# HI-ComputerVision/uni-encoder-code

Hardware: AMD Instinct MI355X
Metric: img/s fwd+bwd Swin-L 1024x2048 bs=2 per GPU (higher is better)
Workload: dtype bf16; 1 GPU; BASELINE configs[2]: full OneFormer (Swin-L ws12 backbone + MSDeformAttn pixel decoder + 150-query masked-attention decoder), 1024x2048, fwd+bwd, synthetic loss; global_batch=2, parallelism=dp1, mode=eval() (train_mode reported separately with --full)

## Files before the change

### include/uenc.h

```cpp
#ifndef UENC_H
#define UENC_H
#include <stdint.h>

#ifdef __cplusplus
extern "C" {
#endif

#define UENC_F32 0
#define UENC_BF16 1

#ifndef UENC_STREAM_T
#define UENC_STREAM_T void*
#endif
typedef UENC_STREAM_T uenc_stream_t;

#define UENC_EPI_NONE 0
#define UENC_EPI_GELU 1
#define UENC_EPI_RELU 2
#define UENC_EPI_RESIDUAL 3
#define UENC_EPI_MUL_DGELU 4
#define UENC_EPI_MUL_DRELU 5

int uenc_version(void);
const char* uenc_arch(void);

int uenc_cast_f32_bf16(const float* src, void* dst, long n , uenc_stream_t stream);
int uenc_dropout_bf16(const void* in, void* out, long n, unsigned seed, float p, uenc_stream_t stream);
int uenc_cast_transpose_f32_bf16(const float* src , void* dst , int R, int C, uenc_stream_t stream);

int uenc_cast_multi(const void* table, int n, long total_tiles, uenc_stream_t stream);

int uenc_upsample_bilinear(const float* in, float* out, long NC, int Hi, int Wi, int Ho, int Wo, uenc_stream_t stream);

int uenc_attn_mask(const float* logits, uint8_t* mask, long rows, int Hi, int Wi, int Ho, int Wo, uenc_stream_t stream);

int uenc_add_cast_bf16(const float* a, const float* b, void* out, long n, long period, uenc_stream_t stream);
int uenc_msda_prep_fwd(const float* offaw, long ld, const float* ref, int ref_per_image, const int64_t* shapes, float* loc,
                       float* aw, long rows, int Lq, int M, int L, int P, uenc_stream_t stream);
int uenc_msda_prep_bwd(const float* dloc, const float* daw, const float* aw, const int64_t* shapes, void* doffaw, long ld,
                       long rows, int Lq, int M, int L, int P, uenc_stream_t stream);
int uenc_segment_colsum(const void* x16, long ld, int cols, const int64_t* seg_start, int nseg, long rows_per_image, int images,
                        float* out, uenc_stream_t stream);

long uenc_groupnorm_tokens_scratch_bytes(int B, int HW, int C, int G);
int uenc_groupnorm_tokens_fwd(const void* x, int x_dtype, const float* gamma, const float* beta, void* y, int y_dtype,
                              float* stats, void* scratch, const float* add_src, int Hs, int Ws, int H, int W, int B, int HW,
                              int C, int G, float eps, int relu, uenc_stream_t stream);
int uenc_groupnorm_tokens_bwd(const void* dy, int dy_dtype, const void* x, int x_dtype, const float* gamma, const float* beta,
                              const float* stats, void* dx, int dx_dtype, float* dgamma, float* dbeta, void* scratch, int B,
                              int HW, int C, int G, int relu, uenc_stream_t stream);
int uenc_upsample_bilinear_tokens_bwd(const void* dy, int dy_dtype, float* dsrc, int B, int H, int W, int Hs, int Ws, int C,
                                      uenc_stream_t stream);
int uenc_im2col3x3(const void* in, void* col, int B, int H, int W, int C, uenc_stream_t stream);
int uenc_col2im3x3(const void* dcol, void* dx, int B, int H, int W, int C, uenc_stream_t stream);
int uenc_im2col3x3_s2(const void* in, void* col, int B, int H, int W, int C, uenc_stream_t stream);
int uenc_col2im3x3_s2(const void* dcol, float* dx, int B, int H, int W, int C, uenc_stream_t stream);

int uenc_gemm_nt(const void* A, int a_dtype, long lda, const void* W, long ldw, void* C, int c_dtype, long ldc,
                 int M, int N, int K, const float* bias, int epilogue, const void* aux, long ldaux,
                 void* aux_out, long ldaux_out, float alpha, int splitk, int accumulate, uenc_stream_t stream);
#define UENC_NT_TILE_256X256 256
#define UENC_NT_TILE_256X192 192
#define UENC_NT_TILE_128X256 128
int uenc_gemm_nt_tile(const void* A, int a_dtype, long lda, const void* W, long ldw, void* C, int c_dtype, long ldc,
                      int M, int N, int K, const float* bias, int epilogue, const void* aux, long ldaux,
                      void* aux_out, long ldaux_out, float alpha, int splitk, int accumulate, int tile, uenc_stream_t stream);
int uenc_gemm_nt_scaled(const void* A, int a_dtype, long lda, const void* W, long ldw, void* C, int c_dtype, long ldc,
                        int M, int N, int K, const float* bias, int epilogue, const void* aux, long ldaux,
                        void* aux_out, long ldaux_out, float alpha, const float* sample_scale, int rows_per_sample, uenc_stream_t stream);
int uenc_gemm_nt_ln(const void* A, int a_dtype, long lda, const void* W, long ldw, void* C, long ldc, int M, int N, int K, const float* bias,
                    const void* residual, long ldres, const float* gamma, const float* beta, float eps, float* y32, void* y16, float* stats,
                    uenc_stream_t stream);
int uenc_gemm_nt_splits(int K, int splitk);
int uenc_gemm_nt_partials(const void* A, int a_dtype, long lda, const void* W, long ldw, float* P, long ldp, long part_stride,
                          int M, int N, int K, float alpha, int splitk, uenc_stream_t stream);

int uenc_gemm_nt_batched(const void* A, int a_dtype, long lda, long bsA, const void* W, long ldw, long bsW, void* C, int c_dtype,
                         long ldc, long bsC, int batch, int M, int N, int K, float alpha, int splitk, int accumulate, uenc_stream_t stream);

int uenc_gemm_tn(const void* dY, int dy_dtype, long ldy, const void* X, int x_dtype, long ldx, float* dW, long ldw,
                 float* db, int M, int N, int K, int splitm, uenc_stream_t stream);
int uenc_gemm_tn_tile(const void* dY, int dy_dtype, long ldy, const void* X, int x_dtype, long ldx, float* dW, long ldw,
                      float* db, int M, int N, int K, int splitm, int tile, uenc_stream_t stream);
int uenc_gemm_tn_scaled(const void* dY, int dy_dtype, long ldy, const void* X, int x_dtype, long ldx, float* dW, long ldw,
                        float* db, int M, int N, int K, int splitm, float alpha, uenc_stream_t stream);

int uenc_gemm_tn_grouped(const void* table, int n, int total_items, int tile, double flops, uenc_stream_t stream);
int uenc_gemm_tn_grouped_small(const void* table, int n, int total_items, double flops, uenc_stream_t stream);

int uenc_layernorm_fwd(const void* x, int x_dtype, const void* res, int res_dtype, float* h_out, const float* gamma,
                       const float* beta, void* y, int y_dtype, float* stats, long M, int C, float eps, void* y16,
                       uenc_stream_t stream);
int uenc_layernorm_bwd(const void* dy, int dy_dtype, const void* h, int h_dtype, const float* stats, const float* gamma,
                       const float* dres, void* dx, int dx_dtype, float* dgamma, float* dbeta, long M, int C, void* dx16,
                       float* part_ws, int defer_param_sums, uenc_stream_t stream);
int uenc_layernorm_bwd_blocks(long M, int C);
int uenc_ln_param_grouped(const void* table, int n, int total_groups, uenc_stream_t stream);
int uenc_patch_merge_ln_fwd(const float* x, const float* gamma, const float* beta, void* y, float* stats, int B, int H, int W,
                            int C, float eps, uenc_stream_t stream);
int uenc_patch_merge_ln_bwd(const void* dy, int dy_dtype, const float* x, const float* stats, const float* gamma, float* dx,
                            float* dgamma, float* dbeta, float* part_ws, int B, int H, int W, int C, int defer_param_sums,
                            uenc_stream_t stream);

int uenc_window_attn_np(int ws);
int uenc_relpos_expand(const float* table , float* bias_q ,
                       float* bias_k , int nH, int ws, uenc_stream_t stream);
int uenc_relpos_expand_grouped(const void* table, int n, int total_blocks, uenc_stream_t stream);
int uenc_window_attn_fwd(const void* qkv, const void* qkv_bias, const float* bias_q, void* out, float* lse, int B, int H, int W,
                         int C, int nH, int ws, int shift, float scale, uenc_stream_t stream);
long uenc_window_attn_bwd_ws_floats(int B, int H, int W, int nH, int ws);
int uenc_window_attn_bwd(const void* qkv, const void* qkv_bias, const float* bias_q, const float* bias_k,
                         const void* o_saved, const float* lse , const void* d_out, void* dqkv,
                         float* dS_ws, float* dtable, float* dbias_pad,
                         int B, int H, int W, int C, int nH, int ws, int shift, float scale, int defer_dtable, uenc_stream_t stream);
int uenc_window_attn_bwd_groups(int B, int H, int W, int nH, int ws);
int uenc_window_attn_dtable_grouped(const void* table, int n, int total_blocks, uenc_stream_t stream);

int uenc_msdeform_attn_fwd(const void* value, int v_dtype, const int64_t* shapes, const int64_t* level_start,
                           const float* loc, const float* attn, void* out, int out_dtype, int B, int S, int M, int D,
                           int L, int Lq, int P, uenc_stream_t stream);
int uenc_msdeform_attn_fwd_tiled(const void* value, int v_dtype, const int64_t* shapes, const int64_t* level_start,
                                 const float* loc, const float* attn, void* out, int out_dtype, int B, int S, int M, int D,
                                 int L, int Lq, int P, const int64_t* shapes_host, uenc_stream_t stream);
int uenc_msdeform_attn_bwd(const void* value, int v_dtype, const int64_t* shapes, const int64_t* level_start,
                           const float* loc, const float* attn, const void* grad_out, int go_dtype, float* grad_value,
                           float* grad_loc, float* grad_attn, int B, int S, int M, int D, int L, int Lq, int P,
                           const int64_t* shapes_host, void* workspace, long workspace_bytes, uenc_stream_t stream);
long uenc_msdeform_attn_bwd_workspace_bytes(const int64_t* shapes_host, int B, int M, int D, int L, int Lq, int P);
int uenc_msdeform_attn_fused_fwd(const void* value, int v_dtype, const int64_t* shapes, const int64_t* level_start, const float* offaw,
                                 long ld, const float* ref, int ref_per_image, void* out, int out_dtype, int B, int S, int M, int D,
                                 int L, int Lq, int P, uenc_stream_t stream);
int uenc_msdeform_attn_fused_fwd_tiled(const void* value, int v_dtype, const int64_t* shapes, const int64_t* level_start, const float* offaw,
                                       long ld, const float* ref, int ref_per_image, void* out, int out_dtype, int B, int S, int M, int D,
                                       int L, int Lq, int P, const int64_t* shapes_host, uenc_stream_t stream);
int uenc_msdeform_attn_fused_bwd(const void* value, int v_dtype, const int64_t* shapes, const int64_t* level_start, const float* offaw,
                                 long ld, const float* ref, int ref_per_image, const void* grad_out, int go_dtype, float* grad_value,
                                 void* doffaw, long ld_doffaw, int B, int S, int M, int D, int L, int Lq, int P, const int64_t* shapes_host,
                                 void* workspace, long workspace_bytes, uenc_stream_t stream);

long uenc_mha_fwd_workspace_floats(int B, int H, int Lq, int S);
int uenc_mha_fwd(const void* q, long q_bs, long q_rs, const void* k, long k_bs, long k_rs, const void* v, long v_bs,
                 long v_rs, const unsigned char* mask, long mask_rs, void* out, long o_bs, long o_rs, float* lse,
                 float* workspace, int B, int H, int Lq, int S, float scale, float dropout_p, unsigned seed, uenc_stream_t stream);
int uenc_mha_bwd(const void* q, long q_bs, long q_rs, const void* k, long k_bs, long k_rs, const void* v, long v_bs,
                 long v_rs, const unsigned char* mask, long mask_rs, const void* out, long o_bs, long o_rs,
                 const float* lse, const void* dout, long do_bs, long do_rs, float* dq, long dq_bs, long dq_rs, void* dk,
                 long dk_bs, long dk_rs, void* dv, long dv_bs, long dv_rs, int B, int H, int Lq, int S, float scale,
                 float dropout_p, unsigned seed, uenc_stream_t stream);

int uenc_na2d_fwd(const void* qkv, const float* rpb, void* out, float* lse, int B, int H, int W, int nH, int K, int dilation,
                  float scale, uenc_stream_t stream);
int uenc_na2d_bwd(const void* qkv, const float* rpb, const void* out, const void* dout, const float* lse, void* dqkv, float* drpb,
                  float* delta_ws, int B, int H, int W, int nH, int K, int dilation, float scale, uenc_stream_t stream);

int uenc_postproc_semantic(const float* mask_logits, const float* class_prob, float* sem, int Q, int C, int Cp, int hl, int wl,
                           int Hp, int Wp, int Ho, int Wo, uenc_stream_t stream);
int uenc_postproc_panoptic_stats(const float* mask_logits, const float* score, int* ids, int* counts, int Q, int hl, int wl, int Hp,
                                 int Wp, int Ho, int Wo, uenc_stream_t stream);
int uenc_postproc_panoptic_label(const float* mask_logits, const int* ids, const int* segid, int* seg, int Q, int hl, int wl, int Hp,
                                 int Wp, int Ho, int Wo, uenc_stream_t stream);

int uenc_gemm_nt_f32(const float* A, long lda, const float* W, long ldw, float* C, long ldc, int M, int N, int K, const float* bias,
                     int epilogue, const float* aux, long ldaux, float* aux_out, long ldaux_out, float alpha, int accumulate, uenc_stream_t stream);
int uenc_gemm_tn_f32(const float* dY, long ldy, const float* X, long ldx, float* dW, long ldw, float* db, int M, int N, int K, uenc_stream_t stream);
int uenc_window_attn_f32_fwd(const float* qkv, const float* qkv_bias, const float* table, float* out, int B, int H, int W, int C, int nH,
                             int ws, int shift, float scale, uenc_stream_t stream);
int uenc_window_attn_f32_bwd(const float* qkv, const float* qkv_bias, const float* table, const float* dout, float* dqkv, float* dtable,
                             float* dbias_pad, int B, int H, int W, int C, int nH, int ws, int shift, float scale, uenc_stream_t stream);
int uenc_mha_f32_fwd(const float* q, long qs0, long qs1, const float* k, long ks0, long ks1, const float* v, long vs0, long vs1,
                     const uint8_t* mask, long mask_row_stride, float* out, long os0, long os1, float* lse, int B, int nH, int Lq, int S,
                     float scale, float dropout_p, unsigned seed, uenc_stream_t stream);
int uenc_mha_f32_bwd(const float* q, long qs0, long qs1, const float* k, long ks0, long ks1, const float* v, long vs0, long vs1,
                     const uint8_t* mask, long mask_row_stride, const float* out, long os0, long os1, const float* lse, const float* dout,
                     long gos0, long gos1, float* dq, long dqs0, long dqs1, float* dk, long dks0, long dks1, float* dv, long dvs0, long dvs1,
                     float* delta, int B, int nH, int Lq, int S, float scale, float dropout_p, unsigned seed, uenc_stream_t stream);
int uenc_na2d_f32_fwd(const float* qkv, const float* rpb, float* out, float* lse, int B, int H, int W, int nH, int K, int dilation,
                      float scale, uenc_stream_t stream);
int uenc_na2d_f32_bwd(const float* qkv, const float* rpb, const float* out, const float* dout, const float* lse, float* dqkv, float* drpb,
                      int B, int H, int W, int nH, int K, int dilation, float scale, uenc_stream_t stream);

// ... 74 lines not shown
```

### uni-encoder-code_amd/csrc/gemm.hip

```cpp
#include "common.h"
#include "prof.h"

#define BM 128
#define BN 128
#define BK 64
#define GEMM_THREADS 256

enum { EPI_NONE = 0, EPI_GELU = 1, EPI_RELU = 2, EPI_RESIDUAL = 3, EPI_MUL_DGELU = 4, EPI_MUL_DRELU = 5 };

struct GemmNT {
    const void* A; int a_f32; long lda;
    const bf16* W; long ldw;
    void* C; long ldc;
    const float* bias;
    const void* aux; long ldaux;
    bf16* aux_out; long ldaux_out;
    int M, N, K;
    int tiles_m, tiles_n;
    int klen;
    int atomic;
    int persist;
    float alpha;
    const float* sample_scale; float inv_rows;
    long part_stride;
    int splits;
    long bsA, bsW, bsC;
    const float* ln_gamma; const float* ln_beta; float* ln_y32; bf16* ln_y16; float2* ln_stats; float ln_eps;
};

__device__ __forceinline__ float nt_alpha(const GemmNT& p, int m) {
    return p.sample_scale == nullptr ? p.alpha : p.alpha * p.sample_scale[(int)(((float)m + 0.5f) * p.inv_rows)];
}

__device__ __forceinline__ int lds_off(int row, int chunk) { return row * 128 + ((chunk ^ ((row >> 1) & 7)) << 4); }

template <bool F32>
__device__ __forceinline__ u32x4 load_row8(const void* base, long ld, int row, int nrows, int k, int kend, int K) {
    const bool ok = (row < nrows) && (k < kend);
    const int rc = min(row, nrows - 1), kc = min(k, K - 8);
    u32x4 v;
    if (F32) {
        const float* p = (const float*)base + (long)rc * ld + kc;
        const float4 a = *(const float4*)p, b = *(const float4*)(p + 4);
        const bf16x8 r = cvt8(a, b);
        v = *(const u32x4*)&r;
    } else {
        v = *(const u32x4*)((const bf16*)base + (long)rc * ld + kc);
    }
    const u32x4 z = {0u, 0u, 0u, 0u};
    return ok ? v : z;
}

template <int EPI, int OUT_F32>
__global__ __launch_bounds__(GEMM_THREADS) void gemm_nt_kernel(GemmNT p) {
    __shared__ __attribute__((aligned(16))) unsigned char smem[2 * (BM + BN) * BK * 2];
    if (blockIdx.z > 0) {
        p.A = (const char*)p.A + (long)blockIdx.z * p.bsA * (p.a_f32 ? 4 : 2);
        p.W += (long)blockIdx.z * p.bsW;
        p.C = (char*)p.C + (long)blockIdx.z * p.bsC * (OUT_F32 ? 4 : 2);
    }
    if (OUT_F32 && p.part_stride > 0) p.C = (float*)p.C + (long)blockIdx.y * p.part_stride;
    const int t = threadIdx.x, lane = t & 63, wave = t >> 6;
    const int wm = wave >> 1, wn = wave & 1;
    const int tile = xcd_remap(blockIdx.x, gridDim.x);
    const int mt = tile / p.tiles_n, nt = tile - mt * p.tiles_n;
    const int m0 = mt * BM, n0 = nt * BN;
    const int kbeg = blockIdx.y * p.klen;
    const int kend = min(p.K, kbeg + p.klen);
    const int nkt = (kend - kbeg + BK - 1) / BK;

    f32x4 acc[4][4];
#pragma unroll
    for (int i = 0; i < 4; ++i)
#pragma unroll
        for (int j = 0; j < 4; ++j) acc[i][j] = (f32x4){0.f, 0.f, 0.f, 0.f};

    const int srow = t >> 3, schunk = t & 7;
    u32x4 ra[4], rw[4];
    auto gload = [&](int kt) {
        const int k = kbeg + kt * BK + schunk * 8;
#pragma unroll
        for (int i = 0; i < 4; ++i) rw[i] = load_row8<false>(p.W, p.ldw, n0 + srow + 32 * i, p.N, k, kend, p.K);
        if (p.a_f32) {
#pragma unroll
            for (int i = 0; i < 4; ++i) ra[i] = load_row8<true>(p.A, p.lda, m0 + srow + 32 * i, p.M, k, kend, p.K);
        } else {
#pragma unroll
            for (int i = 0; i < 4; ++i) ra[i] = load_row8<false>(p.A, p.lda, m0 + srow + 32 * i, p.M, k, kend, p.K);
        }
    };
    auto lstore = [&](int buf) {
        unsigned char* As = smem + buf * ((BM + BN) * BK * 2);
        unsigned char* Ws = As + BM * BK * 2;
#pragma unroll
        for (int i = 0; i < 4; ++i) {
            *(u32x4*)(As + lds_off(srow + 32 * i, schunk)) = ra[i];
            *(u32x4*)(Ws + lds_off(srow + 32 * i, schunk)) = rw[i];
        }
    };

    gload(0);
    lstore(0);
    __syncthreads();
    const int fr = lane & 15, fg = lane >> 4;
    for (int kt = 0; kt < nkt; ++kt) {
        const int buf = kt & 1;
        if (kt + 1 < nkt) gload(kt + 1);
        const unsigned char* As = smem + buf * ((BM + BN) * BK * 2);
        const unsigned char* Ws = As + BM * BK * 2;
#pragma unroll
        for (int ks = 0; ks < 2; ++ks) {
            bf16x8 wf[4], xf[4];
#pragma unroll
            for (int i = 0; i < 4; ++i) wf[i] = *(const bf16x8*)(Ws + lds_off(wn * 64 + i * 16 + fr, ks * 4 + fg));
#pragma unroll
            for (int j = 0; j < 4; ++j) xf[j] = *(const bf16x8*)(As + lds_off(wm * 64 + j * 16 + fr, ks * 4 + fg));
#pragma unroll
            for (int i = 0; i < 4; ++i)
#pragma unroll
                for (int j = 0; j < 4; ++j) acc[i][j] = mfma16(wf[i], xf[j], acc[i][j]);
        }
        if (kt + 1 < nkt) lstore(buf ^ 1);
        __syncthreads();
    }

    const bool lead = (blockIdx.y == 0);
    if (p.atomic) {
#pragma unroll
        for (int j = 0; j < 4; ++j) {
            const int m = m0 + wm * 64 + j * 16 + fr;
            if (m >= p.M) continue;
#pragma unroll
            for (int i = 0; i < 4; ++i) {
                const int n = n0 + wn * 64 + i * 16 + 4 * fg;
                if (n >= p.N) continue;
                float* c = (float*)p.C + (long)m * p.ldc + n;
#pragma unroll
                for (int r = 0; r < 4; ++r) {
                    float v = acc[i][j][r];
                    if (p.bias != nullptr && lead) v += p.bias[n + r];
                    atomicAdd(c + r, v * p.alpha);
                }
            }
        }
        return;
    }
    float* T = (float*)smem;
    constexpr int LDT = 132;
    const int erow = t >> 4, ecol = (t & 15) * 8;
#pragma unroll
    for (int h = 0; h < 2; ++h) {
        __syncthreads();
        if (wm == h) {
#pragma unroll
            for (int j = 0; j < 4; ++j)
#pragma unroll
                for (int i = 0; i < 4; ++i) *(f32x4*)(T + (j * 16 + fr) * LDT + wn * 64 + i * 16 + 4 * fg) = acc[i][j];
        }
        __syncthreads();
        const int n = n0 + ecol;
        if (n >= p.N) continue;
        const bool full8 = (n + 8 <= p.N);
        float bv[8] = {0.f, 0.f, 0.f, 0.f, 0.f, 0.f, 0.f, 0.f};
        if (p.bias != nullptr) {
            const float4 b0 = *(const float4*)(p.bias + n);
            bv[0] = b0.x; bv[1] = b0.y; bv[2] = b0.z; bv[3] = b0.w;
// ... 42 lines not shown
                    v[r] = (EPI == EPI_MUL_DGELU) ? v[r] * dgelu_f((float)sv[r]) : (((float)sv[r] > 0.f) ? v[r] : 0.f);
            }
            if (OUT_F32) {
                float* c = (float*)p.C + (long)m * p.ldc + n;
                *(float4*)c = make_float4(v[0], v[1], v[2], v[3]);
                if (full8) *(float4*)(c + 4) = make_float4(v[4], v[5], v[6], v[7]);
            } else {
                bf16x8 o;
#pragma unroll
                for (int r = 0; r < 8; ++r) o[r] = (bf16)v[r];
                bf16* c = (bf16*)p.C + (long)m * p.ldc + n;
                if (full8) *(bf16x8*)c = o;
                else { bf16x4 q4; q4[0] = o[0]; q4[1] = o[1]; q4[2] = o[2]; q4[3] = o[3]; *(bf16x4*)c = q4; }
            }
        }
    }
}


template <int EPI, int OUT_F32>
__device__ __forceinline__ void epilogue8(const GemmNT& p, int m, int n, bool full8, float (&v)[8]) {
    if (EPI == EPI_GELU) {
        if (p.aux_out != nullptr) {
            bf16x8 pre;
#pragma unroll
            for (int r = 0; r < 8; ++r) pre[r] = (bf16)v[r];
            bf16* dst = p.aux_out + (long)m * p.ldaux_out + n;
            if (full8) *(bf16x8*)dst = pre;
            else { bf16x4 q4; q4[0] = pre[0]; q4[1] = pre[1]; q4[2] = pre[2]; q4[3] = pre[3]; *(bf16x4*)dst = q4; }
        }
#pragma unroll
        for (int r = 0; r < 8; ++r) v[r] = gelu_f(v[r]);
    } else if (EPI == EPI_RELU) {
#pragma unroll
        for (int r = 0; r < 8; ++r) v[r] = fmaxf(v[r], 0.f);
    } else if (EPI == EPI_RESIDUAL) {
        const float* rp = (const float*)p.aux + (long)m * p.ldaux + n;
        const float4 r0 = *(const float4*)rp;
        v[0] += r0.x; v[1] += r0.y; v[2] += r0.z; v[3] += r0.w;
        if (full8) { const float4 r1 = *(const float4*)(rp + 4); v[4] += r1.x; v[5] += r1.y; v[6] += r1.z; v[7] += r1.w; }
    } else if (EPI == EPI_MUL_DGELU || EPI == EPI_MUL_DRELU) {
        const bf16* ap = (const bf16*)p.aux + (long)m * p.ldaux + n;
        bf16x8 sv;
        if (full8) sv = *(const bf16x8*)ap;
        else {
            const bf16x4 q4 = *(const bf16x4*)ap;
#pragma unroll
            for (int r = 0; r < 4; ++r) { sv[r] = q4[r]; sv[4 + r] = (bf16)0.f; }
        }
#pragma unroll
        for (int r = 0; r < 8; ++r)
            v[r] = (EPI == EPI_MUL_DGELU) ? v[r] * dgelu_f((float)sv[r]) : (((float)sv[r] > 0.f) ? v[r] : 0.f);
    }
    if (OUT_F32) {
        float* c = (float*)p.C + (long)m * p.ldc + n;
        *(float4*)c = make_float4(v[0], v[1], v[2], v[3]);
        if (full8) *(float4*)(c + 4) = make_float4(v[4], v[5], v[6], v[7]);
    } else {
        bf16x8 o;
#pragma unroll
        for (int r = 0; r < 8; ++r) o[r] = (bf16)v[r];
        bf16* c = (bf16*)p.C + (long)m * p.ldc + n;
        if (full8) *(bf16x8*)c = o;
        else { bf16x4 q4; q4[0] = o[0]; q4[1] = o[1]; q4[2] = o[2]; q4[3] = o[3]; *(bf16x4*)c = q4; }
    }
}

template <int EPI, int OUT_F32, int A_F32>
__global__ __launch_bounds__(256) void gemm_nt_skinny_kernel(GemmNT p) {
    constexpr int LDP = 68;
    __shared__ __attribute__((aligned(16))) float part[4 * 64 * LDP];
    const int t = threadIdx.x, lane = t & 63, wave = t >> 6;
    const int fr = lane & 15, fg = lane >> 4;
    const int mt = blockIdx.x / p.tiles_n, nt = blockIdx.x - mt * p.tiles_n;
    const int m0 = mt * 64, n0 = nt * 64;
    const int per = (((p.K + 31) >> 5) + 3) >> 2;
    const int kb = wave * per * 32, ke = min(p.K, kb + per * 32);

    f32x4 acc[4][4];
#pragma unroll
    for (int i = 0; i < 4; ++i)
#pragma unroll
        for (int j = 0; j < 4; ++j) acc[i][j] = (f32x4){0.f, 0.f, 0.f, 0.f};
    long aoff[4], woff[4];
#pragma unroll
    for (int j = 0; j < 4; ++j) {
        aoff[j] = (long)min(m0 + j * 16 + fr, p.M - 1) * p.lda;
        woff[j] = (long)min(n0 + j * 16 + fr, p.N - 1) * p.ldw;
    }
    const u32x4 z = {0u, 0u, 0u, 0u};
    for (int k = kb; k < ke; k += 128) {
        u32x4 xa[4][4], wa[4][4];
#pragma unroll
        for (int s = 0; s < 4; ++s) {
            const int kk = k + s * 32 + 8 * fg;
            const bool ok = kk < ke;
            const int kc = min(kk, p.K - 8);
#pragma unroll
            for (int j = 0; j < 4; ++j) {
                if (A_F32) {
                    const float* ap = (const float*)p.A + aoff[j] + kc;
                    const float4 a0 = *(const float4*)ap, a1 = *(const float4*)(ap + 4);
                    const bf16x8 r = cvt8(a0, a1);
                    xa[s][j] = ok ? *(const u32x4*)&r : z;
                } else {
                    const u32x4 v = *(const u32x4*)((const bf16*)p.A + aoff[j] + kc);
                    xa[s][j] = ok ? v : z;
                }
                const u32x4 w = *(const u32x4*)(p.W + woff[j] + kc);
                wa[s][j] = ok ? w : z;
            }
        }
#pragma unroll
        for (int s = 0; s < 4; ++s)
#pragma unroll
            for (int i = 0; i < 4; ++i)
#pragma unroll
                for (int j = 0; j < 4; ++j)
                    acc[i][j] = mfma16(*(const bf16x8*)&wa[s][i], *(const bf16x8*)&xa[s][j], acc[i][j]);
    }
    float* mine = part + wave * 64 * LDP;
#pragma unroll
    for (int j = 0; j < 4; ++j)
#pragma unroll
        for (int i = 0; i < 4; ++i) *(f32x4*)(mine + (j * 16 + fr) * LDP + i * 16 + 4 * fg) = acc[i][j];
    __syncthreads();
    const int row = t >> 2, m = m0 + row;
    if (m >= p.M) return;
#pragma unroll
    for (int h = 0; h < 2; ++h) {
        const int c = (t & 3) * 16 + h * 8, n = n0 + c;
        if (n >= p.N) continue;
        const bool full8 = (n + 8 <= p.N);
        float v[8] = {0.f, 0.f, 0.f, 0.f, 0.f, 0.f, 0.f, 0.f};
#pragma unroll
        for (int w = 0; w < 4; ++w) {
            const f32x4 a0 = *(const f32x4*)(part + (w * 64 + row) * LDP + c), a1 = *(const f32x4*)(part + (w * 64 + row) * LDP + c + 4);
#pragma unroll
            for (int r = 0; r < 4; ++r) { v[r] += a0[r]; v[4 + r] += a1[r]; }
        }
        if (p.bias != nullptr) {
            const float4 b0 = *(const float4*)(p.bias + n);
            v[0] += b0.x; v[1] += b0.y; v[2] += b0.z; v[3] += b0.w;
            if (full8) { const float4 b1 = *(const float4*)(p.bias + n + 4); v[4] += b1.x; v[5] += b1.y; v[6] += b1.z; v[7] += b1.w; }
        }
#pragma unroll
        for (int r = 0; r < 8; ++r) v[r] *= nt_alpha(p, m);
        epilogue8<EPI, OUT_F32>(p, m, n, full8, v);
    }
}

#define BM2 256
#define BN2 256
#define T2 512

__device__ __forceinline__ void wait_vmcnt_upto8(int n) {
    if (n >= 8) __builtin_amdgcn_s_waitcnt(0x0f78);
    else if (n == 7) __builtin_amdgcn_s_waitcnt(0x0f77);
    else if (n == 6) __builtin_amdgcn_s_waitcnt(0x0f76);
    else if (n == 5) __builtin_amdgcn_s_waitcnt(0x0f75);
    else if (n == 4) __builtin_amdgcn_s_waitcnt(0x0f74);
    else if (n == 3) __builtin_amdgcn_s_waitcnt(0x0f73);
    else if (n == 2) __builtin_amdgcn_s_waitcnt(0x0f72);
    else if (n == 1) __builtin_amdgcn_s_waitcnt(0x0f71);
    else __builtin_amdgcn_s_waitcnt(0x0f70);
}

template <int EPI, int NI = 4>
__device__ __forceinline__ void nt_epilogue_direct(const GemmNT& p, f32x4 (&acc)[4][8], int mbase, int nbase, int fr, int fg, bool lead) {
    static_assert(NI == 4 || NI == 3, "column groups per wave");
    constexpr int NP = NI / 2;
    constexpr bool ODD = (NI & 1) != 0;
    const int mrow = mbase + fr, ncol = nbase + 4 * fg;
    const int nodd = ncol + (NI - 1) * 16;
    float bv4[4][4];
#pragma unroll
    for (int i = 0; i < NI; ++i) {
        const int n = ncol + i * 16;
        float4 b = make_float4(0.f, 0.f, 0.f, 0.f);
        if (p.bias != nullptr && n < p.N && lead) b = *(const float4*)(p.bias + n);
        bv4[i][0] = b.x; bv4[i][1] = b.y; bv4[i][2] = b.z; bv4[i][3] = b.w;
    }
    const int odd = fg & 1;
    const int n16[2] = {nbase + (0 + odd) * 16 + 4 * (fg - odd), nbase + (2 + odd) * 16 + 4 * (fg - odd)};
    constexpr bool AUX16 = (EPI == EPI_MUL_DGELU || EPI == EPI_MUL_DRELU);
// ... 571 lines not shown
        unsigned char* As = smem + buf * STAGE3 + wave * 1024;
        unsigned char* Ws = As + BM3 * BK3 * 2;
#pragma unroll
        for (int q = 0; q < 2; ++q) __builtin_amdgcn_global_load_lds(asrc[q] + (long)ks * BK3, (lds_void*)(As + q * 4096), 16, 0, 0);
#pragma unroll
        for (int q = 0; q < 4; ++q) __builtin_amdgcn_global_load_lds(wsrc[q] + (long)ks * BK3, (lds_void*)(Ws + q * 4096), 16, 0, 0);
    };
    issue(0, 0);
    if (nks > 1) issue(1, 1);
    const int aoff = lds_off32(fr, fg), boff = lds_off32(wn * 64 + fr, fg);
    int buf = 0;
    for (int s = 0; s < nks; ++s) {
        if (s + 1 < nks) __builtin_amdgcn_s_waitcnt(0x0f76);
        else __builtin_amdgcn_s_waitcnt(0x0f70);
        __builtin_amdgcn_sched_barrier(0);
        __builtin_amdgcn_s_barrier();
        __builtin_amdgcn_sched_barrier(0);
        if (s + 2 < nks) issue(s + 2, buf == 0 ? 2 : buf - 1);
        const unsigned char* As = smem + buf * STAGE3;
        const unsigned char* Ws = As + BM3 * BK3 * 2;
        bf16x8 wf[4], xf[8];
#pragma unroll
        for (int i = 0; i < 4; ++i) wf[i] = *(const bf16x8*)(Ws + i * 1024 + boff);
#pragma unroll
        for (int j = 0; j < 8; ++j) xf[j] = *(const bf16x8*)(As + j * 1024 + aoff);
        __builtin_amdgcn_sched_barrier(0);
#pragma unroll
        for (int i = 0; i < 4; ++i)
#pragma unroll
            for (int j = 0; j < 8; ++j) acc[i][j] = mfma16(wf[i], xf[j], acc[i][j]);
        buf = buf == 2 ? 0 : buf + 1;
    }
    if (!OUT_F32) {
        nt_epilogue_direct<EPI>(p, acc, m0, n0 + wn * 64, fr, fg, true);
        return;
    }
    __syncthreads();
    nt_epilogue_staged<EPI, OUT_F32, T3, 1, 4, LN>(p, acc, smem, m0, n0, 0, wn, t, fr, fg, true);
}

template <int EPI, int OUT_F32, bool LN = false>
static int launch_nt128(GemmNT& p, hipStream_t stream) {
    p.tiles_m = (p.M + BM3 - 1) / BM3; p.tiles_n = (p.N + BN3 - 1) / BN3;
    static bool attr_set = false;
    if (!attr_set) {
        hipError_t e = hipFuncSetAttribute((const void*)gemm_nt128_kernel<EPI, OUT_F32, LN>, hipFuncAttributeMaxDynamicSharedMemorySize, 3 * STAGE3);
        if (e != hipSuccess) return (int)e;
        attr_set = true;
    }
    p.persist = 0;
    hipLaunchKernelGGL((gemm_nt128_kernel<EPI, OUT_F32, LN>), dim3(p.tiles_m * p.tiles_n), dim3(T3), 3 * STAGE3, stream, p);
    return UENC_OK;
}

static int nt_cu_count() {
    static int ncu = 0;
    if (ncu == 0) {
        int dev = 0, v = 0;
        if (hipGetDevice(&dev) == hipSuccess && hipDeviceGetAttribute(&v, hipDeviceAttributeMultiprocessorCount, dev) == hipSuccess && v >= 8) ncu = v / 8 * 8;
        else ncu = 256;
    }
    return ncu;
}

template <int EPI, int OUT_F32, int BNT = BN2, bool LN = false>
static int launch_nt256(GemmNT& p, hipStream_t stream) {
    p.tiles_m = (p.M + BM2 - 1) / BM2; p.tiles_n = (p.N + BNT - 1) / BNT;
    static bool attr_set = false;
    if (!attr_set) {
        hipError_t e = hipFuncSetAttribute((const void*)gemm_nt256_kernel<EPI, OUT_F32, BNT, LN>, hipFuncAttributeMaxDynamicSharedMemorySize, 131072);
        if (e != hipSuccess) return (int)e;
        attr_set = true;
    }
    const int ncu = nt_cu_count();
    const int ntiles = p.tiles_m * p.tiles_n;
    p.persist = (p.splits == 1 && ntiles > ncu) ? 1 : 0;
    hipLaunchKernelGGL((gemm_nt256_kernel<EPI, OUT_F32, BNT, LN>), dim3(p.persist ? ncu : ntiles, p.splits), dim3(T2), 131072, stream, p);
    return UENC_OK;
}

template <int EPI, int OUT_F32>
static int launch_nt_tile128(GemmNT& p, int batch, hipStream_t stream) {
    p.tiles_m = (p.M + BM - 1) / BM; p.tiles_n = (p.N + BN - 1) / BN;
    hipLaunchKernelGGL((gemm_nt_kernel<EPI, OUT_F32>), dim3(p.tiles_m * p.tiles_n, p.splits, batch), dim3(GEMM_THREADS), 0, stream, p);
    return UENC_OK;
}

template <int EPI, int OUT_F32>
static int launch_nt_skinny(GemmNT& p, hipStream_t stream) {
    p.tiles_m = (p.M + 63) / 64; p.tiles_n = (p.N + 63) / 64;
    const dim3 grid(p.tiles_m * p.tiles_n), block(GEMM_THREADS);
    if (p.a_f32) hipLaunchKernelGGL((gemm_nt_skinny_kernel<EPI, OUT_F32, 1>), grid, block, 0, stream, p);
    else hipLaunchKernelGGL((gemm_nt_skinny_kernel<EPI, OUT_F32, 0>), grid, block, 0, stream, p);
    return UENC_OK;
}

static bool nt192_wins(int M, int N) {
    const long ncu = nt_cu_count(), tm = (M + BM2 - 1) / BM2;
    const long r256 = (tm * ((N + 255) / 256) + ncu - 1) / ncu, r192 = (tm * ((N + 191) / 192) + ncu - 1) / ncu;
    return r192 * 90 < r256 * 100;
}

static bool nt128_wins(int M, int N, int K, int c_dtype) {
    if (c_dtype == UENC_BF16 && M > 200000) return false;
    return N > 192 && N <= 288 && K <= 1024;
}

enum NtRoute { NT_REFUSED = -1, NT_TILE128, NT_SKINNY, NT_HALF, NT_256, NT_192 };

static NtRoute nt_route(int M, int N, int K, int batch, int a_dtype, long lda, int c_dtype, int epilogue, bool summed, int klen, int splitk,
                        bool ln, int tile) {
    const bool prefer_half = tile == 0 ? nt128_wins(M, N, K, c_dtype) : tile == UENC_NT_TILE_128X256;
    const bool dma = batch == 1 && a_dtype == UENC_BF16 && K >= 128 && lda % 8 == 0 && N >= 192 && N % 8 == 0;
    const bool k32 = (K % BK != 0) && (K % BK3 == 0) && !summed && prefer_half;
    const long tiles256 = (long)((M + 255) / 256) * ((N + 255) / 256);
    const bool big = dma && ((K % BK == 0) || k32) &&
                     (summed ? (epilogue == EPI_NONE && c_dtype == UENC_F32 && klen % BK == 0 && tiles256 >= 4 && tiles256 * splitk >= 64) : tiles256 >= 160);
    const long htiles = (long)((M + 127) / 128) * ((N + 255) / 256);
    const bool mid = !big && dma && (K % BK == 0) && !summed && htiles >= 96 &&
                     (c_dtype == UENC_F32 ? (epilogue == EPI_NONE || epilogue == EPI_RESIDUAL || epilogue == EPI_RELU) : true);
    if (tile != 0 && !big) return NT_REFUSED;
    if (ln && !(big || mid)) return NT_REFUSED;
    const long tiles128 = (long)((M + BM - 1) / BM) * ((N + BN - 1) / BN);
    if (!big && batch == 1 && !summed && tiles128 <= 32 && K >= 64) return NT_SKINNY;
    if (!(big || mid)) return NT_TILE128;
    if (mid || (!summed && (K % BK3 == 0) && prefer_half)) return NT_HALF;
    if (tile == UENC_NT_TILE_128X256) return NT_REFUSED;
    const bool narrow_ok = !summed && !(ln && N > 192);
    if (tile == UENC_NT_TILE_256X192 && !narrow_ok) return NT_REFUSED;
    return narrow_ok && (tile == 0 ? nt192_wins(M, N) : tile == UENC_NT_TILE_256X192) ? NT_192 : NT_256;
}

template <int EPI, int OUT_F32>
static int launch_nt(NtRoute route, GemmNT& p, int batch, hipStream_t stream) {
    switch (route) {
        case NT_HALF: return launch_nt128<EPI, OUT_F32>(p, stream);
        case NT_256: return launch_nt256<EPI, OUT_F32>(p, stream);
        case NT_192: return launch_nt256<EPI, OUT_F32, 192>(p, stream);
        default: break;
    }
    if constexpr (EPI != EPI_RESIDUAL || OUT_F32) {
        if (route == NT_SKINNY) return launch_nt_skinny<EPI, OUT_F32>(p, stream);
        if (route == NT_TILE128) return launch_nt_tile128<EPI, OUT_F32>(p, batch, stream);
    }
    return UENC_EINVAL;
}

struct NtLn { const float* gamma; const float* beta; float* y32; void* y16; float* stats; float eps; };

static int gemm_nt_impl(const void* A, int a_dtype, long lda, const void* W, long ldw, void* C, int c_dtype, long ldc,
                        int M, int N, int K, const float* bias, int epilogue, const void* aux, long ldaux,
                        void* aux_out, long ldaux_out, float alpha, int splitk, int accumulate, int batch, long bsA, long bsW,
                        long bsC, hipStream_t stream, long part_stride = 0, const float* sample_scale = nullptr, int rows_per_sample = 0,
                        const NtLn* ln = nullptr, int tile = 0) {
    UENC_CHECK_ARG(A && W && C && M > 0 && N > 0 && K > 0);
    UENC_CHECK_ARG(a_dtype == UENC_F32 || a_dtype == UENC_BF16);
    UENC_CHECK_ARG(c_dtype == UENC_F32 || c_dtype == UENC_BF16);
    UENC_CHECK_ARG(K % 8 == 0 && N % 4 == 0 && ldw % 8 == 0 && ldc % 4 == 0);
    UENC_CHECK_ARG(a_dtype == UENC_F32 ? (lda % 4 == 0) : (lda % 8 == 0));
    UENC_CHECK_ARG(((uintptr_t)A & 15) == 0 && ((uintptr_t)W & 15) == 0 && ((uintptr_t)C & 15) == 0);
    UENC_CHECK_ARG(epilogue >= EPI_NONE && epilogue <= EPI_MUL_DRELU);
    UENC_CHECK_ARG(tile == 0 || tile == UENC_NT_TILE_256X256 || tile == UENC_NT_TILE_256X192 || tile == UENC_NT_TILE_128X256);
    if (epilogue >= EPI_RESIDUAL) UENC_CHECK_ARG(aux != nullptr && ldaux % 4 == 0);
    if (splitk < 1) splitk = 1;
    if (splitk > 1 || accumulate) UENC_CHECK_ARG(c_dtype == UENC_F32 && epilogue == EPI_NONE);
    GemmNT p;
    p.A = A; p.a_f32 = (a_dtype == UENC_F32); p.lda = lda;
    p.W = (const bf16*)W; p.ldw = ldw;
    p.C = C; p.ldc = ldc; p.bias = bias; p.aux = aux; p.ldaux = ldaux;
    p.aux_out = (bf16*)aux_out; p.ldaux_out = ldaux_out;
    p.M = M; p.N = N; p.K = K;
    p.tiles_m = 0; p.tiles_n = 0; p.persist = 0;
    const int kt = (K + BK - 1) / BK;
    if (splitk > kt) splitk = kt;
    p.klen = ((kt + splitk - 1) / splitk) * BK;
    splitk = (K + p.klen - 1) / p.klen;
    p.atomic = (splitk > 1 || accumulate) ? 1 : 0;
    p.part_stride = 0; p.splits = splitk;
    const bool partials = part_stride > 0;
    if (partials) {
        UENC_CHECK_ARG(c_dtype == UENC_F32 && epilogue == EPI_NONE && !accumulate && bias == nullptr && batch == 1 && part_stride % 4 == 0);
        p.atomic = 0; p.part_stride = part_stride;
    }
    p.alpha = alpha;
    p.sample_scale = nullptr; p.inv_rows = 0.f;
    if (sample_scale != nullptr) {
        UENC_CHECK_ARG(rows_per_sample > 0 && !p.atomic && !partials && batch == 1 && M < (1 << 22));
        p.sample_scale = sample_scale; p.inv_rows = 1.0f / (float)rows_per_sample;
    }
    p.bsA = bsA; p.bsW = bsW; p.bsC = bsC;
    p.ln_gamma = nullptr; p.ln_beta = nullptr; p.ln_y32 = nullptr; p.ln_y16 = nullptr; p.ln_stats = nullptr; p.ln_eps = 0.f;

    const bool summed = p.atomic || partials;
    const NtRoute route = nt_route(M, N, K, batch, a_dtype, lda, c_dtype, epilogue, summed, p.klen, splitk, ln != nullptr, tile);
    if (route == NT_REFUSED) return UENC_EINVAL;
    const bool dma_kernel = route == NT_HALF || route == NT_256 || route == NT_192;
    if (c_dtype == UENC_F32) UENC_CHECK_ARG(epilogue == EPI_NONE || epilogue == EPI_RESIDUAL || epilogue == EPI_RELU);
    else UENC_CHECK_ARG(epilogue != EPI_RESIDUAL || dma_kernel);
    if (ln != nullptr) {
        UENC_CHECK_ARG(epilogue == EPI_RESIDUAL && c_dtype == UENC_F32 && !summed && N <= 256 && N % 8 == 0 && ldc == N &&
                       ln->gamma && ln->beta && (ln->y32 || ln->y16));
        UENC_CHECK_ARG((((uintptr_t)ln->gamma | (uintptr_t)ln->beta | (uintptr_t)ln->y32 | (uintptr_t)ln->y16) & 15) == 0 && ((uintptr_t)ln->stats & 7) == 0);
        p.ln_gamma = ln->gamma; p.ln_beta = ln->beta; p.ln_y32 = ln->y32; p.ln_y16 = (bf16*)ln->y16; p.ln_stats = (float2*)ln->stats; p.ln_eps = ln->eps;
    }

    const bool prof = uenc_prof_on();
    if (prof) {
        const double mn = (double)M * N;
        double bytes = (double)M * K * (a_dtype == UENC_F32 ? 4 : 2) + (double)N * K * 2 + mn * (c_dtype == UENC_F32 ? 4 : 2);
        if (epilogue == EPI_RESIDUAL) bytes += mn * 4;
        if (epilogue == EPI_MUL_DGELU || epilogue == EPI_MUL_DRELU) bytes += mn * 2;
        if (aux_out != nullptr) bytes += mn * 2;
        uenc_prof_begin(route == NT_HALF ? UENC_PROF_GEMM_NT128 : dma_kernel ? UENC_PROF_GEMM_NT256 : UENC_PROF_GEMM_NT, 2.0 * batch * M * (double)N * K, stream,
                        batch * bytes);
    }
    int rc = UENC_EINVAL;
    if (ln != nullptr) {
        rc = route == NT_HALF ? launch_nt128<EPI_RESIDUAL, 1, true>(p, stream)
                              : route == NT_192 ? launch_nt256<EPI_RESIDUAL, 1, 192, true>(p, stream) : launch_nt256<EPI_RESIDUAL, 1, BN2, true>(p, stream);
    } else {
        switch (epilogue * 2 + (c_dtype == UENC_F32 ? 1 : 0)) {
#define NT_CASE(E, F) case (E) * 2 + (F): rc = launch_nt<E, F>(route, p, batch, stream); break
            NT_CASE(EPI_NONE, 1); NT_CASE(EPI_RESIDUAL, 1); NT_CASE(EPI_RELU, 1);
            NT_CASE(EPI_NONE, 0); NT_CASE(EPI_GELU, 0); NT_CASE(EPI_RELU, 0); NT_CASE(EPI_MUL_DGELU, 0); NT_CASE(EPI_MUL_DRELU, 0);
            NT_CASE(EPI_RESIDUAL, 0);
#undef NT_CASE
            default: break;
        }
    }
    if (prof) uenc_prof_end(stream);
    if (rc != UENC_OK) return rc;
    UENC_LAUNCH_RET();
}

extern "C" int uenc_gemm_nt(const void* A, int a_dtype, long lda, const void* W, long ldw, void* C, int c_dtype, long ldc,
                            int M, int N, int K, const float* bias, int epilogue, const void* aux, long ldaux,
                            void* aux_out, long ldaux_out, float alpha, int splitk, int accumulate, hipStream_t stream) {
    return gemm_nt_impl(A, a_dtype, lda, W, ldw, C, c_dtype, ldc, M, N, K, bias, epilogue, aux, ldaux, aux_out, ldaux_out, alpha, splitk,
                        accumulate, 1, 0, 0, 0, stream);
}

extern "C" int uenc_gemm_nt_tile(const void* A, int a_dtype, long lda, const void* W, long ldw, void* C, int c_dtype, long ldc,
                                 int M, int N, int K, const float* bias, int epilogue, const void* aux, long ldaux,
                                 void* aux_out, long ldaux_out, float alpha, int splitk, int accumulate, int tile, hipStream_t stream) {
    return gemm_nt_impl(A, a_dtype, lda, W, ldw, C, c_dtype, ldc, M, N, K, bias, epilogue, aux, ldaux, aux_out, ldaux_out, alpha, splitk,
                        accumulate, 1, 0, 0, 0, stream, 0, nullptr, 0, nullptr, tile);
}

extern "C" int uenc_gemm_nt_scaled(const void* A, int a_dtype, long lda, const void* W, long ldw, void* C, int c_dtype, long ldc,
                                   int M, int N, int K, const float* bias, int epilogue, const void* aux, long ldaux,
                                   void* aux_out, long ldaux_out, float alpha, const float* sample_scale, int rows_per_sample,
                                   hipStream_t stream) {
    UENC_CHECK_ARG(sample_scale != nullptr && rows_per_sample > 0);
    return gemm_nt_impl(A, a_dtype, lda, W, ldw, C, c_dtype, ldc, M, N, K, bias, epilogue, aux, ldaux, aux_out, ldaux_out, alpha, 1,
                        0, 1, 0, 0, 0, stream, 0, sample_scale, rows_per_sample);
}

extern "C" int uenc_gemm_nt_ln(const void* A, int a_dtype, long lda, const void* W, long ldw, void* C, long ldc, int M, int N, int K, const float* bias,
                               const void* residual, long ldres, const float* gamma, const float* beta, float eps, float* y32, void* y16, float* stats,
                               hipStream_t stream) {
    UENC_CHECK_ARG(residual != nullptr);
    NtLn ln = {gamma, beta, y32, y16, stats, eps};
    return gemm_nt_impl(A, a_dtype, lda, W, ldw, C, UENC_F32, ldc, M, N, K, bias, EPI_RESIDUAL, residual, ldres, nullptr, 0, 1.0f, 1, 0, 1, 0, 0, 0, stream, 0,
                        nullptr, 0, &ln);
}

extern "C" int uenc_gemm_nt_splits(int K, int splitk) {
    const int kt = (K + BK - 1) / BK;
    if (splitk < 1) splitk = 1;
    if (splitk > kt) splitk = kt;
    const int klen = (kt + splitk - 1) / splitk;
    return (kt + klen - 1) / klen;
}

extern "C" int uenc_gemm_nt_partials(const void* A, int a_dtype, long lda, const void* W, long ldw, float* P, long ldp, long part_stride,
                                     int M, int N, int K, float alpha, int splitk, hipStream_t stream) {
    UENC_CHECK_ARG(splitk >= 1 && uenc_gemm_nt_splits(K, splitk) == splitk && part_stride >= (long)(M - 1) * ldp + N);
    return gemm_nt_impl(A, a_dtype, lda, W, ldw, P, UENC_F32, ldp, M, N, K, nullptr, EPI_NONE, nullptr, 0, nullptr, 0, alpha, splitk, 0, 1, 0, 0,
                        0, stream, part_stride);
}

extern "C" int uenc_gemm_nt_batched(const void* A, int a_dtype, long lda, long bsA, const void* W, long ldw, long bsW, void* C, int c_dtype,
                                    long ldc, long bsC, int batch, int M, int N, int K, float alpha, int splitk, int accumulate,
                                    hipStream_t stream) {
    UENC_CHECK_ARG(batch >= 1 && batch <= 65535);
    UENC_CHECK_ARG((bsA * (a_dtype == UENC_F32 ? 4 : 2)) % 16 == 0 && (bsW * 2) % 16 == 0 && (bsC * (c_dtype == UENC_F32 ? 4 : 2)) % 16 == 0);
    return gemm_nt_impl(A, a_dtype, lda, W, ldw, C, c_dtype, ldc, M, N, K, nullptr, EPI_NONE, nullptr, 0, nullptr, 0, alpha, splitk, accumulate,
                        batch, bsA, bsW, bsC, stream);
}

struct GemmTN {
    const void* dY; int dy_f32; long ldy;
    const void* X; int x_f32; long ldx;
    float* dW; long ldw;
    float* db;
    int M, N, K;
    int tiles_n, tiles_k;
    int mlen;
    int store;
    float alpha;
};

__device__ __forceinline__ void transpose8x8(const u32x4 (&in)[8], u32x4 (&out)[8]) {
#pragma unroll
    for (int c = 0; c < 8; ++c) {
#pragma unroll
        for (int w = 0; w < 4; ++w) {
            const unsigned lo = in[2 * w][c >> 1], hi = in[2 * w + 1][c >> 1];
            out[c][w] = __builtin_amdgcn_perm(hi, lo, (c & 1) ? 0x07060302u : 0x05040100u);
        }
    }
}

__device__ __forceinline__ void tn_small_body(const GemmTN& p, int tile, int msplit) {
    __shared__ __attribute__((aligned(16))) unsigned char smem[2 * (BM + BN) * BK * 2];
    const int t = threadIdx.x, lane = t & 63, wave = t >> 6;
    const int wk = wave >> 1, wn = wave & 1;
    const int ntile = tile / p.tiles_k, ktile = tile - ntile * p.tiles_k;
    const int n0 = ntile * BN, k0 = ktile * BM;
    const int mbeg = msplit * p.mlen;
    const int mend = min(p.M, mbeg + p.mlen);
    const int nit = (mend - mbeg + BK - 1) / BK;
// ... 424 lines not shown
```

### uni-encoder-code_amd/csrc/layernorm.hip

```cpp
#include "common.h"
#include <stdlib.h>

struct LnFwd {
    const void* x; int x_f32;
    const void* res; int res_f32;
    float* h_out;
    const float* gamma; const float* beta;
    void* y; int y_f32;
    bf16* y16;
    float2* stats;
    long M; int C; float eps;
    int mgH, mgW, mgC;
};

struct PatchGather {
    long base; bool ok[4];
    __device__ __forceinline__ PatchGather(long row, int H, int W, int C) {
        const int W2 = (W + 1) >> 1, H2 = (H + 1) >> 1;
        const int j = (int)(row % W2);
        const long r2 = row / W2;
        const int i = (int)(r2 % H2);
        const long b = r2 / H2;
        base = ((b * H + 2 * i) * W + 2 * j) * C;
        const bool y1 = 2 * i + 1 < H, x1 = 2 * j + 1 < W;
// ... 270 lines not shown
}

extern "C" int uenc_layernorm_bwd_blocks(long M, int C) {
    if (M <= 0 || C <= 0) return 0;
    bool stored = false;
    const long b = ln_bwd_blocks(M, C, true, &stored);
    return stored ? (int)b : 0;
}

static int ln_bwd_launch(LnBwd& p, float* part_ws, int defer, hipStream_t stream) {
    const long M = p.M; const int C = p.C;
    float* dgamma = p.dgamma; float* dbeta = p.dbeta;
    bool stored = false;
    const long blocks = ln_bwd_blocks(M, C, part_ws != nullptr && dgamma != nullptr, &stored);
    p.part = stored ? part_ws : nullptr;
    const int nv = (C + 255) / 256;
    const size_t shm = (size_t)(C > 2048 ? 1 : 4) * 2 * C * sizeof(float);
    dim3 grid((unsigned)blocks), block(256);
    if (nv <= 1) LN_LAUNCH(bwd, 1, grid, block, shm, stream, p);
    else if (nv <= 2) LN_LAUNCH(bwd, 2, grid, block, shm, stream, p);
    else if (nv <= 4) LN_LAUNCH(bwd, 4, grid, block, shm, stream, p);
    else if (nv <= 8) LN_LAUNCH(bwd, 8, grid, block, shm, stream, p);
    else if (nv <= 16) LN_LAUNCH(bwd, 16, grid, block, shm, stream, p);
    else LN_LAUNCH(bwd, 24, grid, block, shm, stream, p);
    if (p.part != nullptr && !defer)
        hipLaunchKernelGGL(ln_bwd_param_kernel, dim3((2 * C + 63) / 64, 16), dim3(256), 0, stream, (const float*)p.part, (int)blocks, C, dgamma, dbeta);
    UENC_LAUNCH_RET();
}

struct LnParamDesc { const float* part; float* dgamma; float* dbeta; int nblk, C, group_begin, pad; };
__global__ __launch_bounds__(256) void ln_param_grouped_kernel(const LnParamDesc* __restrict__ table, int n) {
    __shared__ float red[4][64];
    int lo = 0, hi = n - 1;
    const int grp = blockIdx.x;
    while (lo < hi) {
        const int mid = (lo + hi + 1) >> 1;
        if (table[mid].group_begin <= grp) lo = mid; else hi = mid - 1;
    }
    const LnParamDesc d = table[lo];
    const int C = d.C, nblk = d.nblk;
    const int col = (grp - d.group_begin) * 64 + (threadIdx.x & 63), r = threadIdx.x >> 6;
    const int per = (nblk + gridDim.y - 1) / gridDim.y, b0 = blockIdx.y * per, b1 = min(nblk, b0 + per);
    float acc = 0.f;
    if (col < 2 * C)
        for (int b = b0 + r; b < b1; b += 4) acc += d.part[(long)b * 2 * C + col];
    red[r][threadIdx.x & 63] = acc;
    __syncthreads();
    if (r == 0 && col < 2 * C) {
        const float v = red[0][threadIdx.x] + red[1][threadIdx.x] + red[2][threadIdx.x] + red[3][threadIdx.x];
        atomicAdd(col < C ? d.dgamma + col : d.dbeta + (col - C), v);
    }
}

extern "C" int uenc_ln_param_grouped(const void* table, int n, int total_groups, hipStream_t stream) {
    UENC_CHECK_ARG(table && n > 0 && total_groups > 0 && ((uintptr_t)table & 7) == 0);
    static_assert(sizeof(LnParamDesc) == 40, "descriptor layout is part of the ABI");
    hipLaunchKernelGGL(ln_param_grouped_kernel, dim3((unsigned)total_groups, 16), dim3(256), 0, stream, (const LnParamDesc*)table, n);
    UENC_LAUNCH_RET();
}


extern "C" int uenc_patch_merge_ln_fwd(const float* x, const float* gamma, const float* beta, void* y, float* stats, int B, int H, int W,
                                       int C, float eps, hipStream_t stream) {
    UENC_CHECK_ARG(x && gamma && beta && y && stats && B > 0 && H > 0 && W > 0 && C > 0 && C % 4 == 0 && 4 * C <= 6144);
    UENC_CHECK_ARG((((uintptr_t)x | (uintptr_t)y) & 15) == 0);
    LnFwd p;
    p.x = x; p.x_f32 = 1; p.res = nullptr; p.res_f32 = 0; p.h_out = nullptr; p.gamma = gamma; p.beta = beta; p.y = y; p.y_f32 = 0;
    p.y16 = nullptr; p.stats = (float2*)stats; p.M = (long)B * ((H + 1) / 2) * ((W + 1) / 2); p.C = 4 * C; p.eps = eps;
    p.mgH = H; p.mgW = W; p.mgC = C;
    return ln_fwd_launch(p, stream);
}

extern "C" int uenc_patch_merge_ln_bwd(const void* dy, int dy_dtype, const float* x, const float* stats, const float* gamma, float* dx,
                                       float* dgamma, float* dbeta, float* part_ws, int B, int H, int W, int C, int defer_param_sums,
                                       hipStream_t stream) {
    UENC_CHECK_ARG(dy && x && stats && gamma && dx && B > 0 && H > 0 && W > 0 && C > 0 && C % 4 == 0 && 4 * C <= 6144);
    UENC_CHECK_ARG((dgamma == nullptr) == (dbeta == nullptr));
    LnBwd p;
    p.dy = dy; p.dy_f32 = (dy_dtype == UENC_F32); p.h = x; p.h_f32 = 1; p.stats = (const float2*)stats; p.gamma = gamma; p.dres = nullptr;
    p.dx = dx; p.dx_f32 = 1; p.dx16 = nullptr; p.dgamma = dgamma; p.dbeta = dbeta;
    p.M = (long)B * ((H + 1) / 2) * ((W + 1) / 2); p.C = 4 * C; p.mgH = H; p.mgW = W; p.mgC = C;
    return ln_bwd_launch(p, part_ws, defer_param_sums, stream);
}
```

### uni-encoder-code_amd/uenc/attention.py

```python
from typing import Optional

import torch

from . import kernels as K
from .capi import check, lib, stream_ptr


def _strided(t: torch.Tensor) -> torch.Tensor:
    if t.dtype != K.adt():
        t = t.to(K.adt())
    if t.stride(2) != 1 or t.stride(1) % 8 or t.stride(0) % 8 or t.data_ptr() % 16:
        t = t.contiguous()
    return t


def _mask_bytes(mask: Optional[torch.Tensor]):
    if mask is None:
        return None, 0
    m = mask.to(torch.uint8) if mask.dtype != torch.bool else mask.view(torch.uint8)
    S = m.shape[-1]
    if S % 4 or not m.is_contiguous():
        Sp = -(-S // 4) * 4
        m = torch.nn.functional.pad(m, (0, Sp - S)).contiguous()
    return m, m.shape[-1]


class MHACoreFn(torch.autograd.Function):
    @staticmethod
    def forward(ctx, q, k, v, nheads, mask, dropout_p=0.0, seed=0):
        q, k, v = _strided(q), _strided(k), _strided(v)
        B, Lq, E = q.shape
        S = k.shape[1]
        assert E == nheads * 32, "the HIP attention kernels are built for head_dim 32"
        scale = 32 ** -0.5
        m8, mrs = _mask_bytes(mask)
        lse = torch.empty((B, nheads, Lq), dtype=torch.float32, device=q.device)
        if K.EXACT:
            if isinstance(seed, K.SeedSlot):
                raise RuntimeError("device-side dropout seeds (ops.device_rng) are not available in the fp32 exact mode")
            out = torch.empty((B, Lq, E), dtype=torch.float32, device=q.device)
            check(lib.uenc_mha_f32_fwd(q.data_ptr(), q.stride(0), q.stride(1), k.data_ptr(), k.stride(0), k.stride(1),
                                       v.data_ptr(), v.stride(0), v.stride(1), m8.data_ptr() if m8 is not None else 0, mrs,
                                       out.data_ptr(), out.stride(0), out.stride(1), lse.data_ptr(), B, nheads, Lq, S, scale, float(dropout_p), int(seed),
                                       stream_ptr()), "mha_f32_fwd")
            ctx.save_for_backward(q, k, v, out, lse, m8 if m8 is not None else torch.empty(0, device=q.device))
            ctx.meta = (nheads, S, scale, mrs, m8 is not None, float(dropout_p), int(seed))
            return out
        out = torch.empty((B, Lq, E), dtype=torch.bfloat16, device=q.device)
        nws = lib.uenc_mha_fwd_workspace_floats(B, nheads, Lq, S)
        ws = torch.empty((nws,), dtype=torch.float32, device=q.device) if nws else None
        args = (q.data_ptr(), q.stride(0), q.stride(1), k.data_ptr(), k.stride(0), k.stride(1),
                v.data_ptr(), v.stride(0), v.stride(1), m8.data_ptr() if m8 is not None else 0, mrs,
                out.data_ptr(), out.stride(0), out.stride(1), lse.data_ptr(),
                ws.data_ptr() if ws is not None else 0, B, nheads, Lq, S, scale, float(dropout_p))
        if isinstance(seed, K.SeedSlot):
            check(lib.uenc_mha_fwd_sp(*args, seed.seeds.data_ptr(), seed.slot, stream_ptr()), "mha_fwd_sp")
        else:
            check(lib.uenc_mha_fwd(*args, int(seed), stream_ptr()), "mha_fwd")
        ctx.save_for_backward(q, k, v, out, lse, m8 if m8 is not None else torch.empty(0, device=q.device))
        ctx.meta = (nheads, S, scale, mrs, m8 is not None, float(dropout_p), seed if isinstance(seed, K.SeedSlot) else int(seed))
        return out

    @staticmethod
    def backward(ctx, dout):
        q, k, v, out, lse, m8 = ctx.saved_tensors
        nheads, S, scale, mrs, has_mask, dropout_p, seed = ctx.meta
        B, Lq, E = q.shape
        dout = _strided(dout)
        if K.EXACT:
            dq = torch.empty((B, Lq, E), dtype=torch.float32, device=q.device)
            dk = torch.zeros((B, S, E), dtype=torch.float32, device=q.device)
            dv = torch.zeros((B, S, E), dtype=torch.float32, device=q.device)
            delta = torch.empty((B, nheads, Lq), dtype=torch.float32, device=q.device)
            check(lib.uenc_mha_f32_bwd(q.data_ptr(), q.stride(0), q.stride(1), k.data_ptr(), k.stride(0), k.stride(1),
                                       v.data_ptr(), v.stride(0), v.stride(1), m8.data_ptr() if has_mask else 0, mrs,
                                       out.data_ptr(), out.stride(0), out.stride(1), lse.data_ptr(),
                                       dout.data_ptr(), dout.stride(0), dout.stride(1),
                                       dq.data_ptr(), dq.stride(0), dq.stride(1), dk.data_ptr(), dk.stride(0), dk.stride(1),
                                       dv.data_ptr(), dv.stride(0), dv.stride(1), delta.data_ptr(), B, nheads, Lq, S, scale, dropout_p, seed,
                                       stream_ptr()), "mha_f32_bwd")
            return dq, dk, dv, None, None, None, None
        dq = torch.zeros((B, Lq, E), dtype=torch.float32, device=q.device)
        dk = torch.empty((B, S, E), dtype=torch.bfloat16, device=q.device)
        dv = torch.empty((B, S, E), dtype=torch.bfloat16, device=q.device)
        args = (q.data_ptr(), q.stride(0), q.stride(1), k.data_ptr(), k.stride(0), k.stride(1),
                v.data_ptr(), v.stride(0), v.stride(1), m8.data_ptr() if has_mask else 0, mrs,
                out.data_ptr(), out.stride(0), out.stride(1), lse.data_ptr(),
                dout.data_ptr(), dout.stride(0), dout.stride(1),
                dq.data_ptr(), dq.stride(0), dq.stride(1), dk.data_ptr(), dk.stride(0), dk.stride(1),
                dv.data_ptr(), dv.stride(0), dv.stride(1), B, nheads, Lq, S, scale, dropout_p)
        if isinstance(seed, K.SeedSlot):
            seed.check()
            check(lib.uenc_mha_bwd_sp(*args, seed.seeds.data_ptr(), seed.slot, stream_ptr()), "mha_bwd_sp")
        else:
            check(lib.uenc_mha_bwd(*args, seed, stream_ptr()), "mha_bwd")
        return dq.to(torch.bfloat16), dk, dv, None, None, None, None


def mha(q, k, v, nheads: int, mask: Optional[torch.Tensor] = None, dropout_p: float = 0.0, seed: int = 0):
    if not q.is_cuda:
        raise RuntimeError("uenc attention runs on the GPU only")
    return MHACoreFn.apply(q, k, v, nheads, mask, dropout_p, seed)


def keep_mask_reference(B: int, nheads: int, Lq: int, S: int, dropout_p: float, seed: int) -> torch.Tensor:
    idx = torch.arange(B * nheads * Lq * S, dtype=torch.int64)
    M = 0xFFFFFFFF
    x = (((idx & M) ^ (((idx >> 32) * 0x9E3779B9) & M)) + seed) & M
    x = x ^ (x >> 16); x = (x * 0x7feb352d) & M
    x = x ^ (x >> 15); x = (x * 0x846ca68b) & M
    x = x ^ (x >> 16)
    thresh = 0 if dropout_p <= 0 else int(float(torch.tensor(dropout_p, dtype=torch.float32)) * 4294967296.0)
    return (x >= thresh).view(B, nheads, Lq, S)
```

### uni-encoder-code_amd/uenc/capi.py

```python
import ctypes
import os

import torch

_HERE = os.path.dirname(os.path.abspath(__file__))
LIB_PATH = os.path.join(_HERE, "libuenc_hip.so")

F32, BF16 = 0, 1
EPI_NONE, EPI_GELU, EPI_RELU, EPI_RESIDUAL, EPI_MUL_DGELU, EPI_MUL_DRELU = range(6)

c_p, c_i, c_l, c_f, c_u, c_d = ctypes.c_void_p, ctypes.c_int, ctypes.c_long, ctypes.c_float, ctypes.c_uint, ctypes.c_double

_SIGNATURES = {
    "uenc_version": [],
    "uenc_prof_enable": [c_i],
    "uenc_prof_collect": [c_i, c_p, c_p, c_p],
    "uenc_prof_collect_bytes": [c_i, c_p],
    "uenc_prof_next_bytes": [ctypes.c_double],
    "uenc_cast_f32_bf16": [c_p, c_p, c_l, c_p],
    "uenc_cast_transpose_f32_bf16": [c_p, c_p, c_i, c_i, c_p],
    "uenc_cast_multi": [c_p, c_i, c_l, c_p],
    "uenc_upsample_bilinear": [c_p, c_p, c_l, c_i, c_i, c_i, c_i, c_p],
    "uenc_attn_mask": [c_p, c_p, c_l, c_i, c_i, c_i, c_i, c_p],
    "uenc_gemm_nt": [c_p, c_i, c_l, c_p, c_l, c_p, c_i, c_l, c_i, c_i, c_i, c_p, c_i, c_p, c_l, c_p, c_l, c_f, c_i, c_i, c_p],
    "uenc_gemm_nt_tile": [c_p, c_i, c_l, c_p, c_l, c_p, c_i, c_l, c_i, c_i, c_i, c_p, c_i, c_p, c_l, c_p, c_l, c_f, c_i, c_i, c_i, c_p],
    "uenc_gemm_nt_scaled": [c_p, c_i, c_l, c_p, c_l, c_p, c_i, c_l, c_i, c_i, c_i, c_p, c_i, c_p, c_l, c_p, c_l, c_f, c_p, c_i, c_p],
    "uenc_gemm_nt_ln": [c_p, c_i, c_l, c_p, c_l, c_p, c_l, c_i, c_i, c_i, c_p, c_p, c_l, c_p, c_p, c_f, c_p, c_p, c_p, c_p],
    "uenc_groupnorm_tokens_scratch_bytes": [c_i, c_i, c_i, c_i],
    "uenc_groupnorm_tokens_fwd": [c_p, c_i, c_p, c_p, c_p, c_i, c_p, c_p, c_p, c_i, c_i, c_i, c_i, c_i, c_i, c_i, c_i, c_f, c_i, c_p],
    "uenc_groupnorm_tokens_bwd": [c_p, c_i, c_p, c_i, c_p, c_p, c_p, c_p, c_i, c_p, c_p, c_p, c_i, c_i, c_i, c_i, c_i, c_p],
    "uenc_upsample_bilinear_tokens_bwd": [c_p, c_i, c_p, c_i, c_i, c_i, c_i, c_i, c_i, c_p],
    "uenc_im2col3x3": [c_p, c_p, c_i, c_i, c_i, c_i, c_p],
    "uenc_col2im3x3": [c_p, c_p, c_i, c_i, c_i, c_i, c_p],
    "uenc_add_cast_bf16": [c_p, c_p, c_p, c_l, c_l, c_p],
    "uenc_msda_prep_fwd": [c_p, c_l, c_p, c_i, c_p, c_p, c_p, c_l, c_i, c_i, c_i, c_i, c_p],
    "uenc_msda_prep_bwd": [c_p, c_p, c_p, c_p, c_p, c_l, c_l, c_i, c_i, c_i, c_i, c_p],
    "uenc_segment_colsum": [c_p, c_l, c_i, c_p, c_i, c_l, c_i, c_p, c_p],
    "uenc_dropout_bf16": [c_p, c_p, c_l, c_u, c_f, c_p],
    "uenc_gemm_nt_splits": [c_i, c_i],
    "uenc_gemm_nt_partials": [c_p, c_i, c_l, c_p, c_l, c_p, c_l, c_l, c_i, c_i, c_i, c_f, c_i, c_p],
    "uenc_gemm_nt_batched": [c_p, c_i, c_l, c_l, c_p, c_l, c_l, c_p, c_i, c_l, c_l, c_i, c_i, c_i, c_i, c_f, c_i, c_i, c_p],
    "uenc_gemm_tn": [c_p, c_i, c_l, c_p, c_i, c_l, c_p, c_l, c_p, c_i, c_i, c_i, c_i, c_p],
    "uenc_gemm_tn_tile": [c_p, c_i, c_l, c_p, c_i, c_l, c_p, c_l, c_p, c_i, c_i, c_i, c_i, c_i, c_p],
    "uenc_gemm_tn_scaled": [c_p, c_i, c_l, c_p, c_i, c_l, c_p, c_l, c_p, c_i, c_i, c_i, c_i, c_f, c_p],
    "uenc_gemm_tn_grouped": [c_p, c_i, c_i, c_i, ctypes.c_double, c_p],
    "uenc_gemm_tn_grouped_small": [c_p, c_i, c_i, ctypes.c_double, c_p],
    "uenc_layernorm_fwd": [c_p, c_i, c_p, c_i, c_p, c_p, c_p, c_p, c_i, c_p, c_l, c_i, c_f, c_p, c_p],
    "uenc_layernorm_bwd": [c_p, c_i, c_p, c_i, c_p, c_p, c_p, c_p, c_i, c_p, c_p, c_l, c_i, c_p, c_p, c_i, c_p],
    "uenc_layernorm_bwd_blocks": [c_l, c_i],
    "uenc_ln_param_grouped": [c_p, c_i, c_i, c_p],
    "uenc_window_attn_bwd_groups": [c_i, c_i, c_i, c_i, c_i],
    "uenc_window_attn_dtable_grouped": [c_p, c_i, c_i, c_p],
    "uenc_msdeform_attn_fwd": [c_p, c_i, c_p, c_p, c_p, c_p, c_p, c_i, c_i, c_i, c_i, c_i, c_i, c_i, c_i, c_p],
    "uenc_msdeform_attn_fwd_tiled": [c_p, c_i, c_p, c_p, c_p, c_p, c_p, c_i, c_i, c_i, c_i, c_i, c_i, c_i, c_i, c_p, c_p],
    "uenc_msdeform_attn_bwd": [c_p, c_i, c_p, c_p, c_p, c_p, c_p, c_i, c_p, c_p, c_p, c_i, c_i, c_i, c_i, c_i, c_i, c_i, c_p, c_p, c_l, c_p],
    "uenc_msdeform_attn_bwd_workspace_bytes": [c_p, c_i, c_i, c_i, c_i, c_i, c_i],
    "uenc_msdeform_attn_fused_fwd": [c_p, c_i, c_p, c_p, c_p, c_l, c_p, c_i, c_p, c_i, c_i, c_i, c_i, c_i, c_i, c_i, c_i, c_p],
    "uenc_msdeform_attn_fused_fwd_tiled": [c_p, c_i, c_p, c_p, c_p, c_l, c_p, c_i, c_p, c_i, c_i, c_i, c_i, c_i, c_i, c_i, c_i, c_p, c_p],
    "uenc_msdeform_attn_fused_bwd": [c_p, c_i, c_p, c_p, c_p, c_l, c_p, c_i, c_p, c_i, c_p, c_p, c_l, c_i, c_i, c_i, c_i, c_i, c_i, c_i, c_p, c_p, c_l, c_p],
    "uenc_mha_fwd_workspace_floats": [c_i, c_i, c_i, c_i],
    "uenc_mha_fwd": [c_p, c_l, c_l, c_p, c_l, c_l, c_p, c_l, c_l, c_p, c_l, c_p, c_l, c_l, c_p, c_p, c_i, c_i, c_i, c_i, c_f, c_f, c_u, c_p],
    "uenc_mha_bwd": [c_p, c_l, c_l, c_p, c_l, c_l, c_p, c_l, c_l, c_p, c_l, c_p, c_l, c_l, c_p, c_p, c_l, c_l, c_p, c_l, c_l,
                     c_p, c_l, c_l, c_p, c_l, c_l, c_i, c_i, c_i, c_i, c_f, c_f, c_u, c_p],
    "uenc_window_attn_np": [c_i],
    "uenc_relpos_expand": [c_p, c_p, c_p, c_i, c_i, c_p],
    "uenc_relpos_expand_grouped": [c_p, c_i, c_i, c_p],
    "uenc_window_attn_fwd": [c_p, c_p, c_p, c_p, c_p, c_i, c_i, c_i, c_i, c_i, c_i, c_i, c_f, c_p],
    "uenc_postproc_semantic": [c_p, c_p, c_p, c_i, c_i, c_i, c_i, c_i, c_i, c_i, c_i, c_i, c_p],
    "uenc_postproc_panoptic_stats": [c_p, c_p, c_p, c_p, c_i, c_i, c_i, c_i, c_i, c_i, c_i, c_p],
    "uenc_postproc_panoptic_label": [c_p, c_p, c_p, c_p, c_i, c_i, c_i, c_i, c_i, c_i, c_i, c_p],
    "uenc_patch_merge_ln_fwd": [c_p, c_p, c_p, c_p, c_p, c_i, c_i, c_i, c_i, c_f, c_p],
    "uenc_patch_merge_ln_bwd": [c_p, c_i, c_p, c_p, c_p, c_p, c_p, c_p, c_p, c_i, c_i, c_i, c_i, c_i, c_p],
    "uenc_im2col3x3_s2": [c_p, c_p, c_i, c_i, c_i, c_i, c_p],
    "uenc_col2im3x3_s2": [c_p, c_p, c_i, c_i, c_i, c_i, c_p],
    "uenc_na2d_fwd": [c_p, c_p, c_p, c_p, c_i, c_i, c_i, c_i, c_i, c_i, c_f, c_p],
    "uenc_na2d_bwd": [c_p, c_p, c_p, c_p, c_p, c_p, c_p, c_p, c_i, c_i, c_i, c_i, c_i, c_i, c_f, c_p],
    "uenc_window_attn_bwd_ws_floats": [c_i, c_i, c_i, c_i, c_i],
    "uenc_step_rng_advance": [c_p, c_p, c_i, c_i, c_p, c_i, c_p, c_i, c_p],
    "uenc_dropout_sp": [c_p, c_p, c_l, c_i, c_p, c_i, c_f, c_p],
    "uenc_upload": [c_p, c_p, c_l, c_p],
    "uenc_prof_active": [],
    "uenc_scale_rows_bf16": [c_p, c_l, c_p, c_l, c_l, c_i, c_p, c_l, c_p],
    "uenc_mha_fwd_sp": [c_p, c_l, c_l, c_p, c_l, c_l, c_p, c_l, c_l, c_p, c_l, c_p, c_l, c_l, c_p, c_p, c_i, c_i, c_i, c_i, c_f, c_f, c_p, c_i, c_p],
    "uenc_mha_bwd_sp": [c_p, c_l, c_l, c_p, c_l, c_l, c_p, c_l, c_l, c_p, c_l, c_p, c_l, c_l, c_p, c_p, c_l, c_l, c_p, c_l, c_l,
                        c_p, c_l, c_l, c_p, c_l, c_l, c_i, c_i, c_i, c_i, c_f, c_f, c_p, c_i, c_p],
    "uenc_gemm_nt_f32": [c_p, c_l, c_p, c_l, c_p, c_l, c_i, c_i, c_i, c_p, c_i, c_p, c_l, c_p, c_l, c_f, c_i, c_p],
    "uenc_gemm_tn_f32": [c_p, c_l, c_p, c_l, c_p, c_l, c_p, c_i, c_i, c_i, c_p],
    "uenc_window_attn_f32_fwd": [c_p, c_p, c_p, c_p, c_i, c_i, c_i, c_i, c_i, c_i, c_i, c_f, c_p],
    "uenc_window_attn_f32_bwd": [c_p, c_p, c_p, c_p, c_p, c_p, c_p, c_i, c_i, c_i, c_i, c_i, c_i, c_i, c_f, c_p],
    "uenc_mha_f32_fwd": [c_p, c_l, c_l, c_p, c_l, c_l, c_p, c_l, c_l, c_p, c_l, c_p, c_l, c_l, c_p, c_i, c_i, c_i, c_i, c_f, c_f, c_u, c_p],
    "uenc_mha_f32_bwd": [c_p, c_l, c_l, c_p, c_l, c_l, c_p, c_l, c_l, c_p, c_l, c_p, c_l, c_l, c_p, c_p, c_l, c_l, c_p, c_l, c_l,
                         c_p, c_l, c_l, c_p, c_l, c_l, c_p, c_i, c_i, c_i, c_i, c_f, c_f, c_u, c_p],
    "uenc_na2d_f32_fwd": [c_p, c_p, c_p, c_p, c_i, c_i, c_i, c_i, c_i, c_i, c_f, c_p],
    "uenc_na2d_f32_bwd": [c_p, c_p, c_p, c_p, c_p, c_p, c_p, c_i, c_i, c_i, c_i, c_i, c_i, c_f, c_p],
    "uenc_window_attn_bwd": [c_p, c_p, c_p, c_p, c_p, c_p, c_p, c_p, c_p, c_p, c_p, c_i, c_i, c_i, c_i, c_i, c_i, c_i, c_f, c_i, c_p],
    "uenc_optim_advance": [c_p, c_d, c_d, c_p],
    "uenc_optim_grad_sqnorm": [c_p, c_i, c_l, c_p, c_i, c_p, c_f, c_p],
    "uenc_optim_adamw_step": [c_p, c_i, c_l, c_p, c_i, c_p, c_d, c_d, c_d, c_p],
    "uenc_match_cost_workspace_floats": [c_i, c_i, c_i, c_i],
    "uenc_match_cost": [c_p, c_i, c_i, c_i, c_i, c_i, c_i, c_i, c_i, c_i, c_f, c_f, c_f, c_f, c_p, c_l, c_p, c_p],
    "uenc_lsap_solve": [c_p, c_i, c_i, c_p],
    "uenc_view_synth_workspace_floats": [c_i, c_i, c_i, c_i, c_i],
    "uenc_view_synth_fwd": [c_p, c_i, c_i, c_i, c_i, c_i, c_i, c_p],
    "uenc_view_synth_bwd": [c_p, c_i, c_i, c_i, c_i, c_i, c_i, c_p, c_l, c_p],
    "uenc_photo_loss_workspace_floats": [c_i, c_i, c_i, c_i],
    "uenc_photo_loss_fwd": [c_p, c_p, c_p, c_p, c_i, c_i, c_i, c_i, c_i, c_i, c_p, c_l, c_p, c_p, c_p],
    "uenc_photo_loss_bwd": [c_p, c_p, c_p, c_p, c_i, c_i, c_i, c_i, c_i, c_i, c_p, c_p],
    "uenc_dwconv7_ln_fwd": [c_p, c_p, c_p, c_p, c_p, c_p, c_p, c_i, c_p, c_i, c_i, c_i, c_i, c_f, c_p],
    "uenc_dwconv7_ln_bwd_data": [c_p, c_i, c_p, c_p, c_p, c_p, c_p, c_p, c_p, c_p, c_p, c_p, c_i, c_i, c_i, c_i, c_i, c_p],
    "uenc_dwconv7_bwd_weight_workspace_bytes": [c_i, c_i, c_i, c_i],
    "uenc_dwconv7_bwd_weight": [c_p, c_p, c_p, c_p, c_p, c_l, c_i, c_i, c_i, c_i, c_p],
    "uenc_layer_scale_grads": [c_p, c_p, c_p, c_p, c_p, c_p, c_p, c_p, c_i, c_i, c_p],
    "uenc_stem7x7_s2_patches": [c_p, c_p, c_i, c_i, c_i, c_i, c_p],
    "uenc_maxpool3x3_s2_fwd": [c_p, c_p, c_p, c_i, c_i, c_i, c_i, c_i, c_p],
    "uenc_maxpool3x3_s2_bwd": [c_p, c_p, c_p, c_i, c_i, c_i, c_i, c_i, c_p],
    "uenc_bn_workspace_floats": [c_l, c_i],
    "uenc_bn_stats": [c_p, c_i, c_l, c_i, c_p, c_p, c_p, c_p, c_p, c_f, c_p, c_l, c_p],
    "uenc_bn_act_fwd": [c_p, c_i, c_p, c_p, c_p, c_p, c_p, c_i, c_p, c_i, c_l, c_i, c_f, c_i, c_p],
    "uenc_bn_act_bwd_reduce": [c_p, c_i, c_p, c_i, c_p, c_i, c_p, c_p, c_l, c_i, c_f, c_i, c_p, c_p, c_p, c_p, c_l, c_p],
    "uenc_bn_act_bwd_apply": [c_p, c_i, c_p, c_i, c_p, c_i, c_p, c_p, c_p, c_p, c_p, c_i, c_p, c_i, c_l, c_i, c_f, c_i, c_i, c_p],
}


class UencError(RuntimeError):
    pass


def _load():
    if not os.path.exists(LIB_PATH):
        raise ImportError(
            f"{LIB_PATH} is missing: build it with `python -c 'import __graft_entry__ as g; g.build()'` "
            "(or `make -C uni-encoder-code_amd/csrc`). The HIP library is mandatory; there is no fallback path.")
# ... 49 lines not shown
```

### uni-encoder-code_amd/uenc/kernels.py

```python
import ctypes
import os
from typing import Optional

import torch

from . import capi
from .capi import BF16, F32, check, dt, lib, ptr, stream_ptr

EPI_NONE, EPI_GELU, EPI_RELU, EPI_RESIDUAL, EPI_MUL_DGELU, EPI_MUL_DRELU = (
    capi.EPI_NONE, capi.EPI_GELU, capi.EPI_RELU, capi.EPI_RESIDUAL, capi.EPI_MUL_DGELU, capi.EPI_MUL_DRELU)
NT_TILE_256X256, NT_TILE_256X192, NT_TILE_128X256 = 256, 192, 128


EXACT = os.environ.get("UENC_EXACT", "0") == "1"


def adt():
    return torch.float32 if EXACT else torch.bfloat16


def _odt(dtype):
    return torch.float32 if (EXACT and dtype == torch.bfloat16) else dtype


# ... 117 lines not shown
    x = _mix32_np(key, np.uint64(1 << 41) | idx).reshape(nb, n_samples)
    dp = (np.float32(1.0) - kp).astype(np.float32)
    thresh = np.array([0 if d <= 0 else (0xFFFFFFFF if d >= 1 else int(float(d) * 4294967296.0)) for d in dp], dtype=np.uint64)
    keep = (kp[:, None] > 0) & (x >= thresh[:, None])
    inv = (np.float32(1.0) / np.where(kp > 0, kp, np.float32(1.0))).astype(np.float32)
    scales = np.where(keep, inv[:, None], np.float32(0.0)).astype(np.float32)
    return scales, seeds


def cast_bf16(src: torch.Tensor, out: Optional[torch.Tensor] = None) -> torch.Tensor:
    assert src.dtype == torch.float32 and src.is_contiguous() and src.is_cuda
    if EXACT:
        return src if out is None else out.copy_(src)
    if out is None:
        out = torch.empty(src.shape, dtype=torch.bfloat16, device=src.device)
    n = src.numel()
    if n % 8 == 0 and src.data_ptr() % 16 == 0:
        check(lib.uenc_cast_f32_bf16(src.data_ptr(), out.data_ptr(), n, stream_ptr()), "cast_f32_bf16")
    else:
        check(lib.uenc_cast_transpose_f32_bf16(src.data_ptr(), out.data_ptr(), 1, n, stream_ptr()), "cast_f32_bf16")
    return out


def cast_transpose_bf16(src: torch.Tensor, out: Optional[torch.Tensor] = None) -> torch.Tensor:
    assert src.dtype == torch.float32 and src.dim() == 2 and src.is_contiguous() and src.is_cuda
    R, C = src.shape
    if EXACT:
        return src.t().contiguous() if out is None else out.copy_(src.t())
    if out is None:
        out = torch.empty((C, R), dtype=torch.bfloat16, device=src.device)
    assert out.dtype == torch.bfloat16 and tuple(out.shape) == (C, R) and out.is_contiguous()
    check(lib.uenc_cast_transpose_f32_bf16(src.data_ptr(), out.data_ptr(), R, C, stream_ptr()), "cast_transpose")
    return out


def gemm_nt(a: torch.Tensor, w: torch.Tensor, *, bias: Optional[torch.Tensor] = None, epilogue: int = EPI_NONE,
            aux: Optional[torch.Tensor] = None, aux_out: Optional[torch.Tensor] = None,
            out: Optional[torch.Tensor] = None, out_dtype=torch.bfloat16, alpha: float = 1.0,
            splitk: int = 1, accumulate: bool = False, sample_scale: Optional[torch.Tensor] = None, rows_per_sample: int = 0,
            tile: int = 0) -> torch.Tensor:
    _mat(a, "a"); _mat(w, "w")
    M, K = a.shape
    N, K2 = w.shape
    if EXACT:
        if sample_scale is not None:
            raise capi.UencError("gemm_nt: the fp32 verification kernels take no per-sample scale")
        return _gemm_nt_exact(a, w, bias, epilogue, aux, aux_out, out, alpha, accumulate)
    if K != K2 or w.dtype != torch.bfloat16:
        raise capi.UencError(f"gemm_nt: a {tuple(a.shape)} vs w {tuple(w.shape)} / {w.dtype}")
    if out is None:
        out = torch.empty((M, N), dtype=out_dtype, device=a.device)
        if splitk > 1 or accumulate:
            out.zero_()
    _mat(out, "out")
    assert out.shape == (M, N)
    if bias is not None:
        assert bias.dtype == torch.float32 and bias.numel() == N and bias.is_contiguous()
    if aux is not None:
        _mat(aux, "aux"); assert aux.shape == (M, N)
        assert aux.dtype == (torch.float32 if epilogue == EPI_RESIDUAL else torch.bfloat16)
    if aux_out is not None:
        _mat(aux_out, "aux_out"); assert aux_out.shape == (M, N) and aux_out.dtype == torch.bfloat16
    if sample_scale is not None:
        assert sample_scale.dtype == torch.float32 and sample_scale.is_cuda and sample_scale.is_contiguous()
        assert rows_per_sample > 0 and sample_scale.numel() * rows_per_sample >= M and splitk == 1 and not accumulate and tile == 0
        check(lib.uenc_gemm_nt_scaled(a.data_ptr(), dt(a), a.stride(0), w.data_ptr(), w.stride(0), out.data_ptr(), dt(out),
                                      out.stride(0), M, N, K, ptr(bias), epilogue, ptr(aux), aux.stride(0) if aux is not None else 0,
                                      ptr(aux_out), aux_out.stride(0) if aux_out is not None else 0, float(alpha), sample_scale.data_ptr(),
                                      int(rows_per_sample), stream_ptr()), "gemm_nt_scaled")
        return out
    if tile != 0:
        check(lib.uenc_gemm_nt_tile(a.data_ptr(), dt(a), a.stride(0), w.data_ptr(), w.stride(0), out.data_ptr(), dt(out),
                                    out.stride(0), M, N, K, ptr(bias), epilogue, ptr(aux), aux.stride(0) if aux is not None else 0,
                                    ptr(aux_out), aux_out.stride(0) if aux_out is not None else 0, float(alpha), int(splitk),
                                    int(accumulate), int(tile), stream_ptr()), "gemm_nt_tile")
        return out
    check(lib.uenc_gemm_nt(a.data_ptr(), dt(a), a.stride(0), w.data_ptr(), w.stride(0), out.data_ptr(), dt(out),
                           out.stride(0), M, N, K, ptr(bias), epilogue, ptr(aux), aux.stride(0) if aux is not None else 0,
                           ptr(aux_out), aux_out.stride(0) if aux_out is not None else 0, float(alpha), int(splitk),
                           int(accumulate), stream_ptr()), "gemm_nt")
    return out


def _gemm_nt_exact(a, w, bias, epilogue, aux, aux_out, out, alpha, accumulate) -> torch.Tensor:
    M, K = a.shape
    N, K2 = w.shape
    f32 = torch.float32
    if K != K2 or a.dtype != f32 or w.dtype != f32:
        raise capi.UencError(f"gemm_nt (exact): a {tuple(a.shape)} {a.dtype} vs w {tuple(w.shape)} {w.dtype}")
    if out is None:
        out = torch.zeros((M, N), dtype=f32, device=a.device) if accumulate else torch.empty((M, N), dtype=f32, device=a.device)
    _mat(out, "out")
    assert out.shape == (M, N) and out.dtype == f32
    for t, name in ((aux, "aux"), (aux_out, "aux_out")):
        if t is not None:
            _mat(t, name); assert t.shape == (M, N) and t.dtype == f32
    if bias is not None:
        assert bias.dtype == f32 and bias.numel() == N and bias.is_contiguous()
    check(lib.uenc_gemm_nt_f32(a.data_ptr(), a.stride(0), w.data_ptr(), w.stride(0), out.data_ptr(), out.stride(0), M, N, K, ptr(bias),
                               epilogue, ptr(aux), aux.stride(0) if aux is not None else 0, ptr(aux_out),
                               aux_out.stride(0) if aux_out is not None else 0, float(alpha), int(accumulate), stream_ptr()), "gemm_nt_f32")
    return out


def gemm_nt_splitk(a: torch.Tensor, w: torch.Tensor, splitk: int, *, alpha: float = 1.0) -> torch.Tensor:
    _mat(a, "a"); _mat(w, "w")
    M, K = a.shape
    N, K2 = w.shape
    if EXACT:
        return _gemm_nt_exact(a, w, None, EPI_NONE, None, None, None, alpha, False)
    if K != K2 or w.dtype != torch.bfloat16:
        raise capi.UencError(f"gemm_nt_splitk: a {tuple(a.shape)} vs w {tuple(w.shape)} / {w.dtype}")
    s = lib.uenc_gemm_nt_splits(K, int(splitk))
    part = torch.empty((s, M, N), dtype=torch.float32, device=a.device)
    check(lib.uenc_gemm_nt_partials(a.data_ptr(), dt(a), a.stride(0), w.data_ptr(), w.stride(0), part.data_ptr(), N, M * N, M, N, K,
                                    float(alpha), s, stream_ptr()), "gemm_nt_partials")
    return part[0] if s == 1 else part.sum(0)


def gemm_nt_batched(a: torch.Tensor, w: torch.Tensor, out: torch.Tensor, *, alpha: float = 1.0, splitk: int = 1, accumulate: bool = False):
    B, M, K = a.shape
    _, N, _ = w.shape
    if EXACT:
        for b in range(B):
            _gemm_nt_exact(a[b], w[b], None, EPI_NONE, None, None, out[b], alpha, accumulate or splitk > 1)
        return out
    assert a.is_cuda and w.dtype == torch.bfloat16 and w.shape == (B, N, K) and out.shape == (B, M, N)
    assert a.stride(2) == 1 and w.stride(2) == 1 and out.stride(2) == 1
    check(lib.uenc_gemm_nt_batched(a.data_ptr(), dt(a), a.stride(1), a.stride(0), w.data_ptr(), w.stride(1), w.stride(0), out.data_ptr(), dt(out),
                                   out.stride(1), out.stride(0), B, M, N, K, float(alpha), int(splitk), int(accumulate), stream_ptr()),
          "gemm_nt_batched")
    return out


def gemm_tn(dy: torch.Tensor, x: torch.Tensor, dw: torch.Tensor, db: Optional[torch.Tensor] = None, splitm: int = 0, alpha: float = 1.0,
            tile: int = 0):
    _mat(dy, "dy"); _mat(x, "x"); _mat(dw, "dw")
    M, N = dy.shape
    M2, K = x.shape
    if M != M2 or dw.dtype != torch.float32 or dw.shape != (N, K):
        raise capi.UencError(f"gemm_tn: dy {tuple(dy.shape)} x {tuple(x.shape)} dw {tuple(dw.shape)}")
    if db is not None:
        assert db.dtype == torch.float32 and db.numel() == N and db.is_contiguous()
    if EXACT:
        assert dy.dtype == torch.float32 and x.dtype == torch.float32 and alpha == 1.0
        check(lib.uenc_gemm_tn_f32(dy.data_ptr(), dy.stride(0), x.data_ptr(), x.stride(0), dw.data_ptr(), dw.stride(0), ptr(db), M, N, K,
                                   stream_ptr()), "gemm_tn_f32")
        return
    if alpha != 1.0:
        assert tile == 0
        check(lib.uenc_gemm_tn_scaled(dy.data_ptr(), dt(dy), dy.stride(0), x.data_ptr(), dt(x), x.stride(0), dw.data_ptr(), dw.stride(0),
                                      ptr(db), M, N, K, int(splitm), float(alpha), stream_ptr()), "gemm_tn_scaled")
        return
    if tile != 0:
        check(lib.uenc_gemm_tn_tile(dy.data_ptr(), dt(dy), dy.stride(0), x.data_ptr(), dt(x), x.stride(0), dw.data_ptr(), dw.stride(0),
                                    ptr(db), M, N, K, int(splitm), int(tile), stream_ptr()), "gemm_tn_tile")
        return
    check(lib.uenc_gemm_tn(dy.data_ptr(), dt(dy), dy.stride(0), x.data_ptr(), dt(x), x.stride(0), dw.data_ptr(), dw.stride(0),
                           ptr(db), M, N, K, int(splitm), stream_ptr()), "gemm_tn")


def gemm_nt_ln(a: torch.Tensor, w: torch.Tensor, bias: Optional[torch.Tensor], residual: torch.Tensor, gamma: torch.Tensor, beta: torch.Tensor,
               eps: float = 1e-5, want_y32: bool = True, want_y16: bool = True):
    M, Kd = a.shape
    N = w.shape[0]
    if (EXACT or a.dtype != torch.bfloat16 or N > 256 or N % 8 or Kd % 64 or os.environ.get("UENC_GEMM_LN", "1") == "0"
            or not (a.stride(1) == 1 and w.stride(1) == 1 and residual.is_contiguous() and residual.dtype == torch.float32)):
        return None
    h = torch.empty((M, N), dtype=torch.float32, device=a.device)
    y32 = torch.empty((M, N), dtype=torch.float32, device=a.device) if want_y32 else None
    y16 = torch.empty((M, N), dtype=torch.bfloat16, device=a.device) if want_y16 else None
    stats = torch.empty((M, 2), dtype=torch.float32, device=a.device)
    rc = lib.uenc_gemm_nt_ln(a.data_ptr(), dt(a), a.stride(0), w.data_ptr(), w.stride(0), h.data_ptr(), N, M, N, Kd, ptr(bias), residual.data_ptr(), N,
                             gamma.data_ptr(), beta.data_ptr(), float(eps), ptr(y32), ptr(y16), stats.data_ptr(), stream_ptr())
    if rc == -1:
        return None
    check(rc, "gemm_nt_ln")
    return h, y32, y16, stats


def layernorm_fwd(x: torch.Tensor, gamma: torch.Tensor, beta: torch.Tensor, *, res: Optional[torch.Tensor] = None,
                  out_dtype=torch.bfloat16, want_h: bool = False, want_stats: bool = True, eps: float = 1e-5,
                  twin: Optional[list] = None):
    C = x.shape[-1]
    assert x.is_cuda and x.is_contiguous() and gamma.dtype == torch.float32 and beta.dtype == torch.float32
    M = x.numel() // C
    out_dtype = _odt(out_dtype)
    if EXACT and twin is not None:
        twin_exact, twin = twin, None
    else:
        twin_exact = None
    y = torch.empty(x.shape, dtype=out_dtype, device=x.device)
    h = torch.empty(x.shape, dtype=torch.float32, device=x.device) if want_h else None
    stats = torch.empty((M, 2), dtype=torch.float32, device=x.device) if want_stats else None
    if res is not None:
        assert res.shape == x.shape and res.is_contiguous()
    y16 = None
    if twin is not None and out_dtype == torch.float32:
        y16 = torch.empty(x.shape, dtype=torch.bfloat16, device=x.device)
        twin.append(y16)
    check(lib.uenc_layernorm_fwd(x.data_ptr(), dt(x), ptr(res), dt(res) if res is not None else 0, ptr(h),
                                 gamma.data_ptr(), beta.data_ptr(), y.data_ptr(), dt(y), ptr(stats), M, C, float(eps),
                                 ptr(y16), stream_ptr()), "layernorm_fwd")
    if twin_exact is not None and out_dtype == torch.float32:
        twin_exact.append(y)
    return y, h, stats


def layernorm_bwd(dy: torch.Tensor, h: torch.Tensor, stats: torch.Tensor, gamma: torch.Tensor, *,
                  dres: Optional[torch.Tensor] = None, dgamma: Optional[torch.Tensor] = None,
                  dbeta: Optional[torch.Tensor] = None, dx_dtype=torch.float32, twin: Optional[list] = None,
                  defer: Optional["SmallReductions"] = None) -> torch.Tensor:
    C = h.shape[-1]
    M = h.numel() // C
    assert dy.is_contiguous() and h.is_contiguous() and dy.shape == h.shape
    dx_dtype = _odt(dx_dtype)
    twin_exact = None
    if EXACT and twin is not None:
        twin_exact, twin = twin, None
    dx = torch.empty(h.shape, dtype=dx_dtype, device=h.device)
    if dres is not None:
        assert dres.dtype == torch.float32 and dres.is_contiguous() and dres.shape == h.shape
    dx16 = None
    if twin is not None and dx_dtype == torch.float32:
        dx16 = torch.empty(h.shape, dtype=torch.bfloat16, device=h.device)
        twin.append(dx16)
    part, deferred = _ln_part(M, C, dgamma, dbeta, h.device, defer)
    check(lib.uenc_layernorm_bwd(dy.data_ptr(), dt(dy), h.data_ptr(), dt(h), stats.data_ptr(), gamma.data_ptr(),
                                 ptr(dres), dx.data_ptr(), dt(dx), ptr(dgamma), ptr(dbeta), M, C, ptr(dx16), ptr(part), int(deferred), stream_ptr()),
          "layernorm_bwd")
    if twin_exact is not None and dx_dtype == torch.float32:
        twin_exact.append(dx)
    return dx


def postproc_semantic(mask_logits: torch.Tensor, class_prob: torch.Tensor, padded_size, out_size) -> torch.Tensor:
    Q, hl, wl = mask_logits.shape
    C = class_prob.shape[1]
    assert mask_logits.dtype == torch.float32 and mask_logits.is_contiguous() and class_prob.shape[0] == Q
    Cp = -(-C // 32) * 32
    P = torch.zeros((Q, Cp), dtype=torch.float32, device=mask_logits.device)
    P[:, :C] = class_prob
    sem = torch.empty((C, out_size[0], out_size[1]), dtype=torch.float32, device=mask_logits.device)
    check(lib.uenc_postproc_semantic(mask_logits.data_ptr(), P.data_ptr(), sem.data_ptr(), Q, C, Cp, hl, wl, padded_size[0], padded_size[1],
                                     out_size[0], out_size[1], stream_ptr()), "postproc_semantic")
    return sem


def postproc_panoptic_stats(mask_logits: torch.Tensor, score: torch.Tensor, padded_size, out_size):
    Q, hl, wl = mask_logits.shape
    assert mask_logits.dtype == torch.float32 and mask_logits.is_contiguous() and score.dtype == torch.float32 and score.numel() == Q
    ids = torch.empty(tuple(out_size), dtype=torch.int32, device=mask_logits.device)
    counts = torch.zeros((3, Q), dtype=torch.int32, device=mask_logits.device)
    check(lib.uenc_postproc_panoptic_stats(mask_logits.data_ptr(), score.contiguous().data_ptr(), ids.data_ptr(), counts.data_ptr(), Q, hl, wl,
                                           padded_size[0], padded_size[1], out_size[0], out_size[1], stream_ptr()), "postproc_panoptic_stats")
    return ids, counts


def postproc_panoptic_label(mask_logits: torch.Tensor, ids: torch.Tensor, segid: torch.Tensor, padded_size) -> torch.Tensor:
    Q, hl, wl = mask_logits.shape
    assert ids.dtype == torch.int32 and segid.dtype == torch.int32 and segid.numel() == Q and ids.is_contiguous()
    seg = torch.empty_like(ids)
    check(lib.uenc_postproc_panoptic_label(mask_logits.data_ptr(), ids.data_ptr(), segid.contiguous().data_ptr(), seg.data_ptr(), Q, hl, wl,
                                           padded_size[0], padded_size[1], ids.shape[0], ids.shape[1], stream_ptr()), "postproc_panoptic_label")
    return seg


def im2col3x3_s2(x16: torch.Tensor) -> torch.Tensor:
    B, H, W, C = x16.shape
    if EXACT and x16.dtype == torch.float32:
        return im2col3x3_s2(x16.contiguous().view(torch.bfloat16)).view(torch.float32)
    assert x16.dtype == torch.bfloat16 and x16.is_contiguous() and C % 8 == 0
    col = torch.empty((B * ((H + 1) // 2) * ((W + 1) // 2), 9 * C), dtype=torch.bfloat16, device=x16.device)
    check(lib.uenc_im2col3x3_s2(x16.data_ptr(), col.data_ptr(), B, H, W, C, stream_ptr()), "im2col3x3_s2")
    return col


def col2im3x3_s2(dcol: torch.Tensor, B: int, H: int, W: int, C: int) -> torch.Tensor:
    if EXACT and dcol.dtype == torch.float32:
        Ho, Wo = (H + 1) // 2, (W + 1) // 2
        d = dcol.view(B, Ho, Wo, 9, C)
        dxp = dcol.new_zeros((B, 2 * Ho + 2, 2 * Wo + 2, C))
        for t in range(9):
            ky, kx = divmod(t, 3)
            dxp[:, ky:ky + 2 * Ho:2, kx:kx + 2 * Wo:2] += d[:, :, :, t]
        return dxp[:, 1:1 + H, 1:1 + W].contiguous()
    assert dcol.dtype == torch.bfloat16 and dcol.is_contiguous() and dcol.shape[1] == 9 * C
    dx = torch.empty((B, H, W, C), dtype=torch.float32, device=dcol.device)
    check(lib.uenc_col2im3x3_s2(dcol.data_ptr(), dx.data_ptr(), B, H, W, C, stream_ptr()), "col2im3x3_s2")
    return dx


def na2d_fwd(qkv: torch.Tensor, rpb: Optional[torch.Tensor], nH: int, ks: int, dilation: int, scale: float, need_lse: bool = True):
    B, H, W, C3 = qkv.shape
    C = C3 // 3
    if rpb is not None:
        assert rpb.dtype == torch.float32 and rpb.is_contiguous() and tuple(rpb.shape) == (nH, 2 * ks - 1, 2 * ks - 1)
    if EXACT:
        assert qkv.dtype == torch.float32 and qkv.is_contiguous() and C == nH * 32, "na2d: head_dim must be 32"
        out = torch.empty((B, H, W, C), dtype=torch.float32, device=qkv.device)
        lse = torch.empty((B, nH, H, W), dtype=torch.float32, device=qkv.device) if need_lse else None
        check(lib.uenc_na2d_f32_fwd(qkv.data_ptr(), ptr(rpb), out.data_ptr(), ptr(lse), B, H, W, nH, ks, dilation, float(scale), stream_ptr()),
              "na2d_f32_fwd")
        return out, lse
    assert qkv.dtype == torch.bfloat16 and qkv.is_contiguous() and C == nH * 32, "na2d: head_dim must be 32"
    out = torch.empty((B, H, W, C), dtype=torch.bfloat16, device=qkv.device)
    lse = torch.empty((B, nH, H, W), dtype=torch.float32, device=qkv.device) if need_lse else None
    check(lib.uenc_na2d_fwd(qkv.data_ptr(), ptr(rpb), out.data_ptr(), ptr(lse), B, H, W, nH, ks, dilation, float(scale), stream_ptr()),
          "na2d_fwd")
    return out, lse


def na2d_bwd(qkv, rpb, out, dout, lse, nH: int, ks: int, dilation: int, scale: float, drpb: Optional[torch.Tensor]):
    B, H, W, C3 = qkv.shape
    if EXACT:
# ... 769 lines not shown
```

### uni-encoder-code_amd/uenc/modeling/transformer_decoder/oneformer_transformer_decoder.py

```python
import logging
from typing import Optional

import torch
from torch import nn
from torch.nn import functional as F

from ... import kernels as K
from ... import ops
from ...d2 import Conv2d, Registry, configurable
from .position_encoding import PositionEmbeddingSine

TRANSFORMER_DECODER_REGISTRY = Registry("TRANSFORMER_MODULE")
TRANSFORMER_DECODER_REGISTRY.__doc__ = "Registry for transformer module in OneFormer."


def build_transformer_decoder(cfg, in_channels, mask_classification=True):
    name = cfg.MODEL.ONE_FORMER.TRANSFORMER_DECODER_NAME
    return TRANSFORMER_DECODER_REGISTRY.get(name)(cfg, in_channels, mask_classification)


class MultiheadAttention(nn.Module):

    def __init__(self, embed_dim, num_heads, dropout=0.0):
        super().__init__()
        self.embed_dim, self.num_heads = embed_dim, num_heads
        self.dropout = float(dropout)
        self.last_seed = None
        self.in_proj_weight = nn.Parameter(torch.empty(3 * embed_dim, embed_dim))
        self.in_proj_bias = nn.Parameter(torch.zeros(3 * embed_dim))
        self.out_proj = nn.Linear(embed_dim, embed_dim)
        nn.init.xavier_uniform_(self.in_proj_weight)

    def forward(self, query, key, value, attn_mask=None, residual=None):
        E = self.embed_dim
        W, b = self.in_proj_weight, self.in_proj_bias
        if query is key:
            qk = ops.linear(query, W, b, rows=(0, 2 * E))
            q, k = qk[..., :E], qk[..., E:]
        else:
            q = ops.linear(query, W, b, rows=(0, E))
            k = ops.linear(key, W, b, rows=(E, 2 * E))
        v = ops.linear(value, W, b, rows=(2 * E, 3 * E))
        if self.training and self.dropout > 0.0:
            self.last_seed = ops.dropout_seed()
            o = ops.attention(q, k, v, self.num_heads, attn_mask, self.dropout, self.last_seed)
        else:
            o = ops.attention(q, k, v, self.num_heads, attn_mask)
        if residual is not None:
            return ops.linear(o, self.out_proj.weight, self.out_proj.bias, residual=residual)
        return ops.linear(o, self.out_proj.weight, self.out_proj.bias, out_dtype=torch.float32)


def _ln(m: nn.LayerNorm, x, **kw):
    return ops.layer_norm(x, m.weight, m.bias, eps=m.eps, **kw)


class SelfAttentionLayer(nn.Module):
    def __init__(self, d_model, nhead, dropout=0.0, activation="relu", normalize_before=False):
        super().__init__()
        assert not normalize_before, "pre-norm is not used by any shipped config"
        self.self_attn = MultiheadAttention(d_model, nhead, dropout=dropout)
        self.norm = nn.LayerNorm(d_model)

    def forward(self, tgt, tgt_mask=None, tgt_key_padding_mask=None, query_pos=None):
        qk = tgt if query_pos is None else tgt + query_pos
        return _ln(self.norm, self.self_attn(qk, qk, tgt, attn_mask=tgt_mask, residual=tgt))


class CrossAttentionLayer(nn.Module):
    def __init__(self, d_model, nhead, dropout=0.0, activation="relu", normalize_before=False):
        super().__init__()
        assert not normalize_before
        self.multihead_attn = MultiheadAttention(d_model, nhead, dropout=dropout)
        self.norm = nn.LayerNorm(d_model)

    def forward(self, tgt, memory, memory_mask=None, memory_key_padding_mask=None, pos=None, query_pos=None, key_in=None):
        q = tgt if query_pos is None else tgt + query_pos
        k = key_in if key_in is not None else (memory if pos is None else memory + pos)
        return _ln(self.norm, self.multihead_attn(q, k, memory, attn_mask=memory_mask, residual=tgt))


class FFNLayer(nn.Module):
    def __init__(self, d_model, dim_feedforward=2048, dropout=0.0, activation="relu", normalize_before=False):
        super().__init__()
        assert not normalize_before and activation == "relu"
        self.linear1 = nn.Linear(d_model, dim_feedforward)
        self.linear2 = nn.Linear(dim_feedforward, d_model)
        self.norm = nn.LayerNorm(d_model)

    def forward(self, tgt):
        h = ops.mlp(tgt, [self.linear1.weight, self.linear1.bias, self.linear2.weight, self.linear2.bias], act="relu", residual=tgt)
        return _ln(self.norm, h)


class MLP(nn.Module):

    def __init__(self, input_dim, hidden_dim, output_dim, num_layers):
        super().__init__()
        self.num_layers = num_layers
        h = [hidden_dim] * (num_layers - 1)
        self.layers = nn.ModuleList(nn.Linear(n, k) for n, k in zip([input_dim] + h, h + [output_dim]))

    def forward(self, x, out_dtype=torch.float32):
        params = []
        for l in self.layers:
            params += [l.weight, l.bias]
        return ops.mlp(x, params, act="relu", out_dtype=out_dtype)


class TransformerDecoderLayer(nn.Module):

    def __init__(self, d_model, nhead, dim_feedforward=2048, dropout=0.1, activation="relu", normalize_before=False):
        super().__init__()
        assert not normalize_before and activation == "relu"
        self.self_attn = MultiheadAttention(d_model, nhead, dropout=dropout)
        self.multihead_attn = MultiheadAttention(d_model, nhead, dropout=dropout)
        self.linear1 = nn.Linear(d_model, dim_feedforward)
        self.linear2 = nn.Linear(dim_feedforward, d_model)
        self.norm1, self.norm2, self.norm3 = nn.LayerNorm(d_model), nn.LayerNorm(d_model), nn.LayerNorm(d_model)
        self.dropout_p = float(dropout)
        self._masks = []

    def _drop(self, t):
        if ops.device_rng_active():
            return ops.device_dropout(t, self.dropout_p)
        keep = 1.0 - self.dropout_p
        mask = torch.rand(t.shape, device=t.device) < keep
        self._masks.append(mask)
        return t * (mask.to(t.dtype) / keep)

    def forward(self, tgt, memory, key_in, query_pos):
        if self.training and self.dropout_p > 0.0:
            self._masks = []
            qk = tgt + query_pos
            tgt = _ln(self.norm1, tgt + self._drop(self.self_attn(qk, qk, tgt)))
            tgt = _ln(self.norm2, tgt + self._drop(self.multihead_attn(tgt + query_pos, key_in, memory)))
            h = self._drop(F.relu(ops.linear(tgt, self.linear1.weight, self.linear1.bias, out_dtype=torch.float32)))
            h = ops.linear(h, self.linear2.weight, self.linear2.bias, out_dtype=torch.float32)
            return _ln(self.norm3, tgt + self._drop(h))
        qk = tgt + query_pos
        tgt = _ln(self.norm1, self.self_attn(qk, qk, tgt, residual=tgt))
        tgt = _ln(self.norm2, self.multihead_attn(tgt + query_pos, key_in, memory, residual=tgt))
        h = ops.mlp(tgt, [self.linear1.weight, self.linear1.bias, self.linear2.weight, self.linear2.bias], act="relu", residual=tgt)
        return _ln(self.norm3, h)


class TransformerDecoder(nn.Module):
    def __init__(self, layer_args, num_layers, norm=None):
        super().__init__()
        self.layers = nn.ModuleList([TransformerDecoderLayer(*layer_args) for _ in range(num_layers)])
        self.num_layers, self.norm = num_layers, norm


class TransformerEncoder(nn.Module):
    def __init__(self, num_layers, norm=None):
        super().__init__()
        if num_layers != 0:
            raise NotImplementedError("ENC_LAYERS is 0 in every shipped config (oneformer_R50_bs16_90k.yaml:33)")
        self.layers = nn.ModuleList()
        self.num_layers, self.norm = num_layers, norm


class Transformer(nn.Module):

    def __init__(self, d_model=512, nhead=8, num_encoder_layers=6, num_decoder_layers=6, dim_feedforward=2048, dropout=0.1,
                 activation="relu", normalize_before=False, return_intermediate_dec=False):
        super().__init__()
        self.encoder = TransformerEncoder(num_encoder_layers, nn.LayerNorm(d_model) if normalize_before else None)
        self.decoder = TransformerDecoder((d_model, nhead, dim_feedforward, dropout, activation, normalize_before),
                                          num_decoder_layers, nn.LayerNorm(d_model))
        for p in self.parameters():
            if p.dim() > 1:
                nn.init.xavier_uniform_(p)
        self.d_model, self.nhead = d_model, nhead

# ... 48 lines not shown
                self.input_proj.append(nn.Sequential())
        self.class_input_proj = Conv2d(in_channels, hidden_dim, kernel_size=1)
        if self.mask_classification:
            self.class_embed = nn.Linear(hidden_dim, num_classes + 1)
        self.mask_embed = MLP(hidden_dim, hidden_dim, mask_dim, 3)
        self._mem_cache = {}
        self.forced_attn_masks = None

    @classmethod
    def from_config(cls, cfg, in_channels, mask_classification):
        of = cfg.MODEL.ONE_FORMER
        assert of.DEC_LAYERS >= 1
        return {"in_channels": in_channels, "mask_classification": mask_classification,
                "num_classes": cfg.MODEL.SEM_SEG_HEAD.NUM_CLASSES, "hidden_dim": of.HIDDEN_DIM,
                "num_queries": of.NUM_OBJECT_QUERIES, "nheads": of.NHEADS, "dim_feedforward": of.DIM_FEEDFORWARD,
                "dec_layers": of.DEC_LAYERS - 1, "class_dec_layers": of.CLASS_DEC_LAYERS, "enc_layers": of.ENC_LAYERS,
                "dropout": of.DROPOUT, "pre_norm": of.PRE_NORM, "enforce_input_project": of.ENFORCE_INPUT_PROJ,
                "is_train": cfg.MODEL.IS_TRAIN, "mask_dim": cfg.MODEL.SEM_SEG_HEAD.MASK_DIM,
                "use_task_norm": of.USE_TASK_NORM}

    @staticmethod
    def _tok(x):
        B, C, H, W = x.shape
        return x.permute(0, 2, 3, 1).reshape(B, H * W, C)

    def forward(self, x, mask_features, tasks, mask=None):
        assert len(x) == self.num_feature_levels
        del mask
        B = mask_features.shape[0]
        dev = mask_features.device
        src, kin, size_list = [], [], []
        for i in range(self.num_feature_levels):
            H, W = x[i].shape[-2:]
            size_list.append((H, W))
            t = self._tok(x[i])
            ip = self.input_proj[i]
            if not (isinstance(ip, nn.Sequential) and len(ip) == 0):
                t = ops.linear(t, ip.weight, ip.bias, out_dtype=torch.float32)
            s = t + self.level_embed.weight[i].view(1, 1, -1)
            src.append(s)
            kin.append(s + self.pe_layer.tokens(B, H, W, dev))
        Q = self.num_queries
        qe = self.query_embed.weight[None].expand(B, -1, -1)
        t_tok = tasks[:, None, :]
        if self.use_task_norm:
            t_tok = _ln(self.decoder_norm, t_tok)

        H4, W4 = mask_features.shape[-2:]
        mf32 = self._tok(mask_features.float())
        if not mf32.is_contiguous():
            mf32 = mf32.contiguous()
        mkey = (B, H4, W4, str(dev))
        mem = self._mem_cache.get(mkey)
        if mem is None:
            self._mem_cache.clear()
            mem = self.pe_layer.tokens(B, H4, W4, dev).contiguous()
            self._mem_cache[mkey] = mem
            if not K.EXACT:
                ops._register_twin(mem, K.cast_bf16(mem.view(-1, mem.shape[-1])))
        key_in = ops.linear(mf32, self.class_input_proj.weight, self.class_input_proj.bias, residual=mem, out_dtype=K.adt())
        tgt = t_tok.expand(-1, Q - 1, -1) if self.use_task_norm else torch.zeros_like(qe[:, :-1])
        out_t = self.class_transformer(mem, key_in, qe[:, :-1], tgt)
        output = torch.cat([out_t, t_tok], 1)
        query_class = output

        mf16 = None if K.EXACT else ops._twin(mf32)
        if mf16 is None:
            mf16 = mf32.detach().to(K.adt())
        mf16_chw = torch.empty((B, mf32.shape[2], mf32.shape[1]), dtype=K.adt(), device=mf32.device)
        for b in range(B):
            K.cast_transpose_bf16(mf32[b].detach(), out=mf16_chw[b])
        mes = []
        predictions_class, predictions_mask = [], []
        cls, msk, attn_mask = self.forward_prediction_heads(output, (mf16, H4, W4, mes), size_list[0])
        predictions_class.append(cls); predictions_mask.append(msk)
        for i in range(self.num_layers):
            lvl = i % self.num_feature_levels
            if self.forced_attn_masks is not None:
                attn_mask = self.forced_attn_masks[i]
                attn_mask = attn_mask & ~attn_mask.all(-1, keepdim=True)
            output = self.transformer_cross_attention_layers[i](output, src[lvl], memory_mask=attn_mask, query_pos=qe,
                                                                key_in=kin[lvl])
            output = self.transformer_self_attention_layers[i](output, query_pos=qe)
            output = self.transformer_ffn_layers[i](output)
            cls, msk, attn_mask = self.forward_prediction_heads(output, (mf16, H4, W4, mes),
                                                                size_list[(i + 1) % self.num_feature_levels])
            predictions_class.append(cls); predictions_mask.append(msk)
        assert len(predictions_class) == self.num_layers + 1
        nq = predictions_class[0].shape[1]
        allc = ops.linear(torch.cat(predictions_class, 1), self.class_embed.weight, self.class_embed.bias, out_dtype=torch.float32)
        predictions_class = [allc[:, i * nq:(i + 1) * nq] for i in range(len(predictions_class))]
        predictions_mask = [m.view(B, -1, H4, W4) for m in ops.mask_heads(mf32, mf16_chw, [m.view(B, -1, H4 * W4) for m in predictions_mask], mes)]
        return {"contrastive_logits": query_class if self.is_train else None,
                "pred_logits": predictions_class[-1], "pred_masks": predictions_mask[-1],
                "aux_outputs": [{"pred_logits": a, "pred_masks": b} for a, b in zip(predictions_class[:-1], predictions_mask[:-1])]}

    def forward_prediction_heads(self, output, mf, attn_mask_target_size):
        mf16, H4, W4, mes = mf
        d = _ln(self.decoder_norm, output)
        outputs_class = d
        me = self.mask_embed(d, out_dtype=torch.bfloat16).contiguous()
        B, Q, _ = me.shape
        mes.append(me)
        outputs_mask = ops.mask_logits_eager(me, mf16).view(B, Q, H4, W4)
        am = K.attn_mask(outputs_mask.detach(), attn_mask_target_size)
        return outputs_class, outputs_mask, am
```

### uni-encoder-code_amd/uenc/ops.py

```python
import copy
import os
import weakref
from typing import List, Optional, Sequence, Tuple

import torch
import torch.nn.functional as F

from . import kernels as K

BF16, F32 = torch.bfloat16, torch.float32


class ParamCache:

    def __init__(self):
        self._store = {}
        self.casts = 0
        self._table = None

    def invalidate(self):
        self._store.clear()
        self._table = None

    def _get(self, p: torch.Tensor, kind, make, plan=None):
# ... 573 lines not shown
        inputs, pres = [h], []
        for i in range(n):
            w, b = params[2 * i], params[2 * i + 1]
            if i < n - 1:
                if act == "gelu":
                    pre = torch.empty((h.shape[0], w.shape[0]), dtype=K.adt(), device=h.device)
                    h = _fwd_gemm(h, w, b, None, epilogue=K.EPI_GELU, aux_out=pre)
                    pres.append(pre)
                else:
                    h = _fwd_gemm(h, w, b, None, epilogue=K.EPI_RELU)
                inputs.append(h)
            else:
                if residual is not None:
                    r2 = residual.reshape(-1, w.shape[0]).contiguous()
                    out = _fwd_gemm(h, w, b, None, epilogue=K.EPI_RESIDUAL, aux=r2, out_dtype=F32)
                else:
                    out = _fwd_gemm(h, w, b, None, out_dtype=out_dtype)
        ctx.save_for_backward(*inputs, *pres, *params)
        ctx.n, ctx.act, ctx.has_res, ctx.xshape, ctx.xdtype = n, act, residual is not None, x.shape, x.dtype
        return out.reshape(*x.shape[:-1], out.shape[-1])

    @staticmethod
    def backward(ctx, dy):
        n, act = ctx.n, ctx.act
        sv = ctx.saved_tensors
        inputs = sv[:n]
        npre = n - 1 if act == "gelu" else 0
        pres = sv[n:n + npre]
        params = sv[n + npre:]
        g = dy.reshape(-1, dy.shape[-1])
        if g.stride(1) != 1 or (g.stride(0) % 8) != 0:
            g = g.contiguous()
        dx = None
        for i in reversed(range(n)):
            w, b = params[2 * i], params[2 * i + 1]
            _wgrad(g, inputs[i], w, b)
            if i > 0:
                if act == "gelu":
                    g = _dgrad_gemm(g, w, None, epilogue=K.EPI_MUL_DGELU, aux=pres[i - 1])
                else:
                    g = _dgrad_gemm(g, w, None, epilogue=K.EPI_MUL_DRELU, aux=inputs[i])
            elif ctx.needs_input_grad[0]:
                dx = _dgrad_gemm(g, w, None, out_dtype=ctx.xdtype).reshape(ctx.xshape)
        return (dx, (dy if ctx.has_res else None), None, None) + (None,) * len(params)


def mlp(x, params: Sequence[torch.Tensor], *, act="relu", residual=None, out_dtype=BF16):
    return MLPFn.apply(x, residual, act, out_dtype, *params)


class LayerNormFn(torch.autograd.Function):
    @staticmethod
    def forward(ctx, x, res, gamma, beta, out_dtype, eps):
        xc = x.contiguous()
        rc = res.contiguous() if res is not None else None
        need_h = rc is not None or xc.dtype != F32
        tw = [] if (out_dtype == F32 and xc.numel() // xc.shape[-1] >= _BIG_M) else None
        y, h, stats = K.layernorm_fwd(xc, gamma.detach(), beta.detach(), res=rc, out_dtype=out_dtype, want_h=need_h, eps=eps, twin=tw)
        if tw:
            _register_twin(y, tw[0])
        ctx.save_for_backward(h if need_h else xc, stats, gamma, beta)
        ctx.has_res, ctx.xdtype, ctx.rdtype = rc is not None, x.dtype, (res.dtype if res is not None else None)
        return y

    @staticmethod
    def backward(ctx, dy):
        h, stats, gamma, beta = ctx.saved_tensors
        dg = grad_buf(gamma) if gamma.requires_grad else None
        db = grad_buf(beta) if gamma.requires_grad else None
        tw = [] if h.numel() // h.shape[-1] >= _BIG_M else None
        dx = _ln_bwd(dy.contiguous(), h, stats, gamma.detach(), dgamma=dg, dbeta=db, twin=tw)
        if tw:
            _register_twin(dx, tw[0])
        _tn_notify(gamma, beta)
        dxx = dx if ctx.xdtype == F32 else dx.to(ctx.xdtype)
        dr = None
        if ctx.has_res:
            dr = dx if ctx.rdtype == F32 else dx.to(ctx.rdtype)
        return dxx, dr, None, None, None, None


def layer_norm(x, gamma, beta, *, res=None, out_dtype=F32, eps=1e-5):
    return LayerNormFn.apply(x, res, gamma, beta, out_dtype, eps)


class DeviceScales:
    __slots__ = ("vec", "owner", "gen")

    def __init__(self, vec: torch.Tensor, owner=None):
        self.vec, self.owner = vec, owner
        self.gen = owner.generation if owner is not None else 0

    def check(self):
        if self.owner is not None and self.owner.generation != self.gen:
            raise RuntimeError("device RNG: ops.begin_step() ran between this DropPath branch's forward and its backward -- the table "
                               "now holds the next step's multipliers")

    def __len__(self):
        return self.vec.numel()


class DeviceRNG:
    MAX_BRANCH = 1024
    MAX_SEED = 1024

    def __init__(self, seed: int, device=None):
        self.device = torch.device("cuda", torch.cuda.current_device()) if device is None else torch.device(device)
        self.state = torch.tensor([int(seed) & (2 ** 63 - 1), 0], dtype=torch.int64, device=self.device)
        self.keep_prob = torch.ones(self.MAX_BRANCH, dtype=F32, device=self.device)
        self.seeds = torch.zeros(self.MAX_SEED, dtype=torch.int32, device=self.device)
        self.scales = None
        self.n_samples = 0
        self.branch_keep = []
        self.n_seed = 0
        self._nb = self._ns = 0
        self.generation = 0

    def _launch(self, advance: bool):
        nb = len(self.branch_keep) if self.scales is not None else 0
        K.step_rng_advance(self.state, self.keep_prob, nb, max(self.n_samples, 1), self.scales if nb else self.keep_prob, self.n_seed,
                           self.seeds, advance)

    def begin_step(self):
        self._nb = self._ns = 0
        self.generation += 1
        self._launch(True)

    def _register(self, what: str):
        if torch.cuda.is_current_stream_capturing():
            raise RuntimeError(f"device RNG: a new {what} slot was claimed during stream capture -- run one step eagerly first so that every "
                               "slot is registered")

    def claim_branch(self, B: int, keep: float) -> DeviceScales:
        i = self._nb
        self._nb += 1
        if self.scales is None:
            self.n_samples = int(B)
            self.scales = torch.zeros(self.MAX_BRANCH * self.n_samples, dtype=F32, device=self.device)
        if B != self.n_samples:
            raise ValueError(f"device RNG: batch size {B} differs from the {self.n_samples} its tables were laid out for")
        if i == len(self.branch_keep):
            self._register("DropPath")
            if i >= self.MAX_BRANCH:
                raise RuntimeError(f"device RNG: more than {self.MAX_BRANCH} DropPath branches")
            self.branch_keep.append(float(keep))
            self.keep_prob[i].fill_(float(keep))
            self._launch(False)
        elif self.branch_keep[i] != float(keep):
            raise RuntimeError(f"device RNG: DropPath slot {i} was registered with keep probability {self.branch_keep[i]}, now {keep}")
        return DeviceScales(self.scales[i * B:(i + 1) * B], self)

    def claim_seed(self) -> K.SeedSlot:
        j = self._ns
        self._ns += 1
        if j == self.n_seed:
            self._register("dropout seed")
            if j >= self.MAX_SEED:
                raise RuntimeError(f"device RNG: more than {self.MAX_SEED} dropout sites")
            self.n_seed += 1
            self._launch(False)
        return K.SeedSlot(self.seeds, j, self)

    def get_state(self) -> torch.Tensor:
        return self.state.clone()

    def set_state(self, state: torch.Tensor):
# ... 412 lines not shown
            if not t.is_cuda:
                raise RuntimeError("Not implemented on the CPU")
            if not t.is_contiguous():
                raise RuntimeError("tensor has to be contiguous")
        ctx.shapes_host = _host_shapes(value_spatial_shapes)
        out = K.msdeform_attn_fwd(value, value_spatial_shapes, value_level_start_index, sampling_locations,
                                  attention_weights, out_dtype=out_dtype or (F32 if value.dtype == F32 else BF16), shapes_host=ctx.shapes_host)
        ctx.save_for_backward(value, value_spatial_shapes, value_level_start_index, sampling_locations, attention_weights)
        return out

    @staticmethod
    def backward(ctx, grad_output):
        value, shapes, start, loc, attn = ctx.saved_tensors
        gv, gl, ga = K.msdeform_attn_bwd(value, shapes, start, loc, attn, grad_output.contiguous(), ctx.shapes_host)
        return (gv if value.dtype == F32 else gv.to(value.dtype)), None, None, gl, ga, None, None


def mask_logits_eager(me, mf16_tok):
    B, Q, C = me.shape
    HW = mf16_tok.shape[1]
    assert HW % 8 == 0 and C % 8 == 0
    out = torch.empty((B, Q, HW), dtype=F32, device=me.device)
    med = me.detach()
    for b in range(B):
        K.gemm_nt(med[b], mf16_tok[b], out=out[b])
    return out


class MaskHeadsFn(torch.autograd.Function):

    @staticmethod
    def forward(ctx, mf32_tok, mf16_chw, pre, *mes):
        ctx.save_for_backward(mf16_chw, *mes)
        ctx.shape = tuple(mf32_tok.shape)
        return tuple(pre)

    @staticmethod
    def backward(ctx, *douts):
        mf16_chw, *mes = ctx.saved_tensors
        B, HW, C = ctx.shape
        n, Q = len(mes), mes[0].shape[1]
        Mp = -(-(n * Q) // 64) * 64
        dev = mf16_chw.device
        D = torch.empty((B, Mp, HW), dtype=K.adt(), device=dev)
        ME = torch.zeros((B, Mp, C), dtype=K.adt(), device=dev)
        for h, (d, me) in enumerate(zip(douts, mes)):
            r = h * Q
            if d is None:
                D[:, r:r + Q].zero_()
                continue
            d = d if d.is_contiguous() else d.contiguous()
            for b in range(B):
                K.cast_bf16(d[b], out=D[b, r:r + Q])
            ME[:, r:r + Q] = me
        if n * Q < Mp:
            D[:, n * Q:].zero_()
        tiles = -(-Mp // 256) * -(-C // 256)
        split = max(1, min(HW // 512, -(-256 // tiles)))
        dme = [K.gemm_nt_splitk(D[b], mf16_chw[b], split) for b in range(B)]
        dmf = None
        if ctx.needs_input_grad[0] and K.EXACT:
            dmf = torch.zeros((B, HW, C), dtype=F32, device=dev)
            for b in range(B):
                K.gemm_tn(D[b], ME[b], dmf[b], None)
        elif ctx.needs_input_grad[0]:
            dmf = torch.empty((B, HW, C), dtype=F32, device=dev)
            tile = 256 if C % 256 == 0 else 128
            tiles_k = -(-C // tile)
            items = -(-HW // tile) * tiles_k
            WgradQueue.launch(tile, [(D[b].data_ptr(), ME[b].data_ptr(), dmf[b].data_ptr(), 0, D.stride(1), C, C, Mp, HW, C, tiles_k, Mp, 1, items, 1)
                                     for b in range(B)], dev)
        return (dmf, None, None) + tuple(torch.stack([dme[b][h * Q:(h + 1) * Q] for b in range(B)]).to(mes[h].dtype) for h in range(n))


def mask_heads(mf32_tok, mf16_chw, pre, mes):
    return MaskHeadsFn.apply(mf32_tok, mf16_chw, list(pre), *mes)


def attention(q, k, v, nheads: int, mask: Optional[torch.Tensor] = None, dropout_p: float = 0.0, seed: int = 0) -> torch.Tensor:
    from .attention import mha
    return mha(q, k, v, nheads, mask, dropout_p, seed)


class GroupNormTokensFn(torch.autograd.Function):

    @staticmethod
    def forward(ctx, x, gamma, beta, G, eps, relu, add_src, add_hw, out_dtype, dx_dtype):
        xc = x if x.is_contiguous() else x.contiguous()
        src = None
        if add_src is not None:
            src = add_src.float()
            src = src if src.is_contiguous() else src.contiguous()
        y, stats = K.groupnorm_tokens_fwd(xc, gamma.detach(), beta.detach(), G, eps, relu=relu, add_src=src, add_hw=add_hw,
                                          out_dtype=out_dtype)
        ctx.save_for_backward(xc, gamma, beta, stats)
        ctx.cfg = (G, relu, add_hw, None if add_src is None else tuple(add_src.shape), dx_dtype)
        return y

    @staticmethod
    def backward(ctx, dy):
        x, gamma, beta, stats = ctx.saved_tensors
        G, relu, add_hw, src_shape, dx_dtype = ctx.cfg
        dy = dy if dy.is_contiguous() else dy.contiguous()
        train = gamma.requires_grad
        dx = K.groupnorm_tokens_bwd(dy, x, gamma.detach(), beta.detach(), stats, G, relu=relu,
                                    dgamma=grad_buf(gamma) if train else None, dbeta=grad_buf(beta) if train else None,
                                    dx_dtype=dx_dtype)
        if train:
            _tn_notify(gamma, beta)
        dsrc = None
        if src_shape is not None and ctx.needs_input_grad[6]:
            B, Hs, Ws, C = src_shape
            dsrc = K.upsample_bilinear_tokens_bwd(dy.view(B, add_hw[0], add_hw[1], C), Hs, Ws)
        return dx, None, None, None, None, None, dsrc, None, None, None


def group_norm_tokens(x, gn, *, relu=False, add_src=None, add_hw=None, out_dtype=F32, dx_dtype=BF16):
    assert not (relu and add_src is not None)
    return GroupNormTokensFn.apply(x, gn.weight, gn.bias, gn.num_groups, gn.eps, relu, add_src, add_hw, out_dtype, dx_dtype)


def _conv_wmat(weight, tag, transposed=False, pad8=False):
    def make():
        w = weight.detach().permute(0, 2, 3, 1).reshape(weight.shape[0], -1)
        if pad8:
            w = F.pad(w, (0, -w.shape[1] % 8, 0, -w.shape[0] % 8))
        w = w.contiguous()
        return K.cast_transpose_bf16(w) if transposed else K.cast_bf16(w)
    return CACHE._get(weight, tag + "t" if transposed else tag, make)


def _conv_dy(dy, M, Co):
    dy2 = dy.reshape(M, Co)
    dy2 = dy2 if dy2.is_contiguous() else dy2.contiguous()
    return dy2 if dy2.dtype == K.adt() else K.cast_bf16(dy2.float())


def _conv_wgrad(dy2, col, weight, bias, gemm=None):
    Co, C, kh, kw = weight.shape
    dw = torch.zeros((dy2.shape[1], col.shape[1]), dtype=F32, device=dy2.device)
    db = torch.zeros((dy2.shape[1],), dtype=F32, device=dy2.device) if bias is not None else None
    (gemm or K.gemm_tn)(dy2, col, dw, db)
    grad_buf(weight).add_(dw[:Co, :kh * kw * C].view(Co, kh, kw, C).permute(0, 3, 1, 2))
    if bias is not None:
        grad_buf(bias).add_(db[:Co])
    _tn_notify(weight, bias)


class Conv3x3Fn(torch.autograd.Function):

    @staticmethod
    def _wgrad_gemm(dy2, col, dw, db):
        M, Co = dy2.shape
        Kd = col.shape[1]
        if M % 64 == 0 and Co % 8 == 0 and not K.EXACT:
            tile = 256 if Co % 256 == 0 else 128
            nsplit = max(1, M // 16384)
            mlen = -(-(M // 64) // nsplit) * 64
            nsplit = -(-M // mlen)
            tiles_k = -(-Kd // tile)
            WgradQueue.launch(tile, [(dy2.data_ptr(), col.data_ptr(), dw.data_ptr(), 0, Co, Kd, Kd, M, Co, Kd, tiles_k, mlen,
                                      nsplit, -(-Co // tile) * tiles_k * nsplit, 0)], dy2.device)
        else:
            K.gemm_tn(dy2, col, dw, None)

    @staticmethod
# ... 476 lines not shown
```

Before: 30.34 img/s.

## Fuse query-pos add into QKV GEMM and chain decoder LayerNorms

Adds a GEMM variant that adds a second f32 operand (the query positional embedding, broadcast by period) to A while loading tiles, only for the Q/K columns. This lets decoder self-attention skip materialising tgt+query_pos. It also adds a fused two-LayerNorm kernel, forward and backward, so the FFN output norm and the decoder_norm for the prediction heads run in one pass. These changes target small launches and memory traffic in the 150-query decoder, at the cost of new kernel variants and more complex autograd paths.

```diff
diff --git a/include/uenc.h b/include/uenc.h
--- a/include/uenc.h
+++ b/include/uenc.h
@@ -71,6 +71,10 @@
 int uenc_gemm_nt_ln(const void* A, int a_dtype, long lda, const void* W, long ldw, void* C, long ldc, int M, int N, int K, const float* bias,
                     const void* residual, long ldres, const float* gamma, const float* beta, float eps, float* y32, void* y16, float* stats,
                     uenc_stream_t stream);
+int uenc_gemm_nt_adda(const void* A, int a_dtype, long lda, const void* W, long ldw, void* C, int c_dtype, long ldc,
+                      int M, int N, int K, const float* bias, int epilogue, const void* aux, long ldaux,
+                      void* aux_out, long ldaux_out, float alpha, int splitk, int accumulate, const float* a2, long lda2,
+                      int a2_period, int n_add, uenc_stream_t stream);
 int uenc_gemm_nt_splits(int K, int splitk);
 int uenc_gemm_nt_partials(const void* A, int a_dtype, long lda, const void* W, long ldw, float* P, long ldp, long part_stride,
                           int M, int N, int K, float alpha, int splitk, uenc_stream_t stream);
@@ -96,6 +100,13 @@
                        float* part_ws, int defer_param_sums, uenc_stream_t stream);
 int uenc_layernorm_bwd_blocks(long M, int C);
 int uenc_ln_param_grouped(const void* table, int n, int total_groups, uenc_stream_t stream);
+int uenc_layernorm2_fwd(const void* x, int x_dtype, const void* res, int res_dtype, float* h_out, const float* gamma_a,
+                        const float* beta_a, float eps_a, float* y, float* stats_a, const float* gamma_b, const float* beta_b,
+                        float eps_b, float* d32, void* d16, float* stats_b, long M, int C, uenc_stream_t stream);
+int uenc_layernorm2_bwd(const void* dd, int dd_dtype, const float* y, const float* stats_b, const float* gamma_b, const float* dy,
+                        const void* h, int h_dtype, const float* stats_a, const float* gamma_a, const float* dres, float* dx,
+                        void* dx16, float* dgamma_a, float* dbeta_a, float* dgamma_b, float* dbeta_b, long M, int C,
+                        float* part_ws_a, float* part_ws_b, int defer_param_sums, uenc_stream_t stream);
 int uenc_patch_merge_ln_fwd(const float* x, const float* gamma, const float* beta, void* y, float* stats, int B, int H, int W,
                             int C, float eps, uenc_stream_t stream);
 int uenc_patch_merge_ln_bwd(const void* dy, int dy_dtype, const float* x, const float* stats, const float* gamma, float* dx,
diff --git a/uni-encoder-code_amd/csrc/gemm.hip b/uni-encoder-code_amd/csrc/gemm.hip
--- a/uni-encoder-code_amd/csrc/gemm.hip
+++ b/uni-encoder-code_amd/csrc/gemm.hip
@@ -26,6 +26,7 @@
     int splits;
     long bsA, bsW, bsC;
     const float* ln_gamma; const float* ln_beta; float* ln_y32; bf16* ln_y16; float2* ln_stats; float ln_eps;
+    const float* a2; long lda2; int a2_period; int n_add;
 };
 
 __device__ __forceinline__ float nt_alpha(const GemmNT& p, int m) {
@@ -51,7 +52,22 @@
     return ok ? v : z;
 }
 
-template <int EPI, int OUT_F32>
+__device__ __forceinline__ u32x4 load_row8_add(const void* base, long ld, const float* a2, long lda2, int period, int row, int nrows, int k,
+                                               int kend, int K) {
+    const bool ok = (row < nrows) && (k < kend);
+    const int rc = min(row, nrows - 1), kc = min(k, K - 8);
+    const float* p = (const float*)base + (long)rc * ld + kc;
+    const float* q = a2 + (long)(rc % period) * lda2 + kc;
+    float4 a = *(const float4*)p, b = *(const float4*)(p + 4);
+    const float4 c = *(const float4*)q, d = *(const float4*)(q + 4);
+    a.x += c.x; a.y += c.y; a.z += c.z; a.w += c.w;
+    b.x += d.x; b.y += d.y; b.z += d.z; b.w += d.w;
+    const bf16x8 r = cvt8(a, b);
+    const u32x4 z = {0u, 0u, 0u, 0u};
+    return ok ? *(const u32x4*)&r : z;
+}
+
+template <int EPI, int OUT_F32, bool ADDA = false>
 __global__ __launch_bounds__(GEMM_THREADS) void gemm_nt_kernel(GemmNT p) {
     __shared__ __attribute__((aligned(16))) unsigned char smem[2 * (BM + BN) * BK * 2];
     if (blockIdx.z > 0) {
@@ -81,7 +97,11 @@
         const int k = kbeg + kt * BK + schunk * 8;
 #pragma unroll
         for (int i = 0; i < 4; ++i) rw[i] = load_row8<false>(p.W, p.ldw, n0 + srow + 32 * i, p.N, k, kend, p.K);
-        if (p.a_f32) {
+        if (ADDA && n0 < p.n_add) {
+#pragma unroll
+            for (int i = 0; i < 4; ++i)
+                ra[i] = load_row8_add(p.A, p.lda, p.a2, p.lda2, p.a2_period, m0 + srow + 32 * i, p.M, k, kend, p.K);
+        } else if (p.a_f32) {
 #pragma unroll
             for (int i = 0; i < 4; ++i) ra[i] = load_row8<true>(p.A, p.lda, m0 + srow + 32 * i, p.M, k, kend, p.K);
         } else {
@@ -290,11 +310,14 @@
     for (int i = 0; i < 4; ++i)
 #pragma unroll
         for (int j = 0; j < 4; ++j) acc[i][j] = (f32x4){0.f, 0.f, 0.f, 0.f};
-    long aoff[4], woff[4];
+    long aoff[4], woff[4], a2off[4];
+    const bool adda = (A_F32 == 2) && n0 < p.n_add;
 #pragma unroll
     for (int j = 0; j < 4; ++j) {
-        aoff[j] = (long)min(m0 + j * 16 + fr, p.M - 1) * p.lda;
+        const int mr = min(m0 + j * 16 + fr, p.M - 1);
+        aoff[j] = (long)mr * p.lda;
         woff[j] = (long)min(n0 + j * 16 + fr, p.N - 1) * p.ldw;
+        a2off[j] = (A_F32 == 2) ? (long)(mr % p.a2_period) * p.lda2 : 0;
     }
     const u32x4 z = {0u, 0u, 0u, 0u};
     for (int k = kb; k < ke; k += 128) {
@@ -308,7 +331,13 @@
             for (int j = 0; j < 4; ++j) {
                 if (A_F32) {
                     const float* ap = (const float*)p.A + aoff[j] + kc;
-                    const float4 a0 = *(const float4*)ap, a1 = *(const float4*)(ap + 4);
+                    float4 a0 = *(const float4*)ap, a1 = *(const float4*)(ap + 4);
+                    if (adda) {
+                        const float* bp = p.a2 + a2off[j] + kc;
+                        const float4 b0 = *(const float4*)bp, b1 = *(const float4*)(bp + 4);
+                        a0.x += b0.x; a0.y += b0.y; a0.z += b0.z; a0.w += b0.w;
+                        a1.x += b1.x; a1.y += b1.y; a1.z += b1.z; a1.w += b1.w;
+                    }
                     const bf16x8 r = cvt8(a0, a1);
                     xa[s][j] = ok ? *(const u32x4*)&r : z;
                 } else {
@@ -1046,7 +1075,9 @@
 template <int EPI, int OUT_F32>
 static int launch_nt_tile128(GemmNT& p, int batch, hipStream_t stream) {
     p.tiles_m = (p.M + BM - 1) / BM; p.tiles_n = (p.N + BN - 1) / BN;
-    hipLaunchKernelGGL((gemm_nt_kernel<EPI, OUT_F32>), dim3(p.tiles_m * p.tiles_n, p.splits, batch), dim3(GEMM_THREADS), 0, stream, p);
+    const dim3 grid(p.tiles_m * p.tiles_n, p.splits, batch), block(GEMM_THREADS);
+    if (p.a2 != nullptr) hipLaunchKernelGGL((gemm_nt_kernel<EPI, OUT_F32, true>), grid, block, 0, stream, p);
+    else hipLaunchKernelGGL((gemm_nt_kernel<EPI, OUT_F32>), grid, block, 0, stream, p);
     return UENC_OK;
 }
 
@@ -1054,7 +1085,8 @@
 static int launch_nt_skinny(GemmNT& p, hipStream_t stream) {
     p.tiles_m = (p.M + 63) / 64; p.tiles_n = (p.N + 63) / 64;
     const dim3 grid(p.tiles_m * p.tiles_n), block(GEMM_THREADS);
-    if (p.a_f32) hipLaunchKernelGGL((gemm_nt_skinny_kernel<EPI, OUT_F32, 1>), grid, block, 0, stream, p);
+    if (p.a2 != nullptr) hipLaunchKernelGGL((gemm_nt_skinny_kernel<EPI, OUT_F32, 2>), grid, block, 0, stream, p);
+    else if (p.a_f32) hipLaunchKernelGGL((gemm_nt_skinny_kernel<EPI, OUT_F32, 1>), grid, block, 0, stream, p);
     else hipLaunchKernelGGL((gemm_nt_skinny_kernel<EPI, OUT_F32, 0>), grid, block, 0, stream, p);
     return UENC_OK;
 }
@@ -1116,7 +1148,7 @@
                         int M, int N, int K, const float* bias, int epilogue, const void* aux, long ldaux,
                         void* aux_out, long ldaux_out, float alpha, int splitk, int accumulate, int batch, long bsA, long bsW,
                         long bsC, hipStream_t stream, long part_stride = 0, const float* sample_scale = nullptr, int rows_per_sample = 0,
-                        const NtLn* ln = nullptr, int tile = 0) {
+                        const NtLn* ln = nullptr, int tile = 0, const float* a2 = nullptr, long lda2 = 0, int a2_period = 0, int n_add = 0) {
     UENC_CHECK_ARG(A && W && C && M > 0 && N > 0 && K > 0);
     UENC_CHECK_ARG(a_dtype == UENC_F32 || a_dtype == UENC_BF16);
     UENC_CHECK_ARG(c_dtype == UENC_F32 || c_dtype == UENC_BF16);
@@ -1154,11 +1186,19 @@
     }
     p.bsA = bsA; p.bsW = bsW; p.bsC = bsC;
     p.ln_gamma = nullptr; p.ln_beta = nullptr; p.ln_y32 = nullptr; p.ln_y16 = nullptr; p.ln_stats = nullptr; p.ln_eps = 0.f;
+    p.a2 = nullptr; p.lda2 = 0; p.a2_period = 1; p.n_add = 0;
 
     const bool summed = p.atomic || partials;
     const NtRoute route = nt_route(M, N, K, batch, a_dtype, lda, c_dtype, epilogue, summed, p.klen, splitk, ln != nullptr, tile);
     if (route == NT_REFUSED) return UENC_EINVAL;
     const bool dma_kernel = route == NT_HALF || route == NT_256 || route == NT_192;
+    if (a2 != nullptr) {
+        UENC_CHECK_ARG(a_dtype == UENC_F32 && !summed && batch == 1 && ln == nullptr && lda2 % 4 == 0 && ((uintptr_t)a2 & 15) == 0);
+        UENC_CHECK_ARG(a2_period > 0 && n_add >= 0 && n_add <= N && (route == NT_SKINNY || route == NT_TILE128));
+        const int ctile = route == NT_SKINNY ? 64 : BN;
+        UENC_CHECK_ARG(n_add % ctile == 0 || n_add == N);
+        if (n_add > 0) { p.a2 = a2; p.lda2 = lda2; p.a2_period = a2_period; p.n_add = n_add; }
+    }
     if (c_dtype == UENC_F32) UENC_CHECK_ARG(epilogue == EPI_NONE || epilogue == EPI_RESIDUAL || epilogue == EPI_RELU);
     else UENC_CHECK_ARG(epilogue != EPI_RESIDUAL || dma_kernel);
     if (ln != nullptr) {
@@ -1202,6 +1242,15 @@
                             void* aux_out, long ldaux_out, float alpha, int splitk, int accumulate, hipStream_t stream) {
     return gemm_nt_impl(A, a_dtype, lda, W, ldw, C, c_dtype, ldc, M, N, K, bias, epilogue, aux, ldaux, aux_out, ldaux_out, alpha, splitk,
                         accumulate, 1, 0, 0, 0, stream);
+}
+
+extern "C" int uenc_gemm_nt_adda(const void* A, int a_dtype, long lda, const void* W, long ldw, void* C, int c_dtype, long ldc,
+                                 int M, int N, int K, const float* bias, int epilogue, const void* aux, long ldaux,
+                                 void* aux_out, long ldaux_out, float alpha, int splitk, int accumulate, const float* a2, long lda2,
+                                 int a2_period, int n_add, hipStream_t stream) {
+    UENC_CHECK_ARG(a2 != nullptr);
+    return gemm_nt_impl(A, a_dtype, lda, W, ldw, C, c_dtype, ldc, M, N, K, bias, epilogue, aux, ldaux, aux_out, ldaux_out, alpha, splitk,
+                        accumulate, 1, 0, 0, 0, stream, 0, nullptr, 0, nullptr, 0, a2, lda2, a2_period, n_add);
 }
 
 extern "C" int uenc_gemm_nt_tile(const void* A, int a_dtype, long lda, const void* W, long ldw, void* C, int c_dtype, long ldc,
diff --git a/uni-encoder-code_amd/csrc/layernorm.hip b/uni-encoder-code_amd/csrc/layernorm.hip
--- a/uni-encoder-code_amd/csrc/layernorm.hip
+++ b/uni-encoder-code_amd/csrc/layernorm.hip
@@ -376,3 +376,279 @@
     p.M = (long)B * ((H + 1) / 2) * ((W + 1) / 2); p.C = 4 * C; p.mgH = H; p.mgW = W; p.mgC = C;
     return ln_bwd_launch(p, part_ws, defer_param_sums, stream);
 }
+
+
+struct Ln2Fwd {
+    const void* x; int x_f32;
+    const void* res; int res_f32;
+    float* h_out;
+    const float* gamma_a; const float* beta_a; float* y; float2* stats_a; float eps_a;
+    const float* gamma_b; const float* beta_b; float* d32; bf16* d16; float2* stats_b; float eps_b;
+    long M; int C;
+};
+
+template <int NV>
+__global__ __launch_bounds__(256) void ln2_fwd_kernel(Ln2Fwd p) {
+    const int lane = threadIdx.x & 63;
+    const long wave0 = (long)blockIdx.x * 4 + (threadIdx.x >> 6);
+    const long nwaves = (long)gridDim.x * 4;
+    const float invC = 1.0f / (float)p.C;
+    for (long row = wave0; row < p.M; row += nwaves) {
+        float4 v[NV];
+        float s = 0.f;
+#pragma unroll
+        for (int i = 0; i < NV; ++i) {
+            const int c = lane * 4 + i * 256;
+            if (c < p.C) {
+                v[i] = load4(p.x, p.x_f32, row * p.C + c);
+                if (p.res != nullptr) {
+                    const float4 r = load4(p.res, p.res_f32, row * p.C + c);
+                    v[i].x += r.x; v[i].y += r.y; v[i].z += r.z; v[i].w += r.w;
+                }
+                if (p.h_out != nullptr) *(float4*)(p.h_out + row * p.C + c) = v[i];
+                s += v[i].x + v[i].y + v[i].z + v[i].w;
+            } else {
+                v[i] = make_float4(0.f, 0.f, 0.f, 0.f);
+            }
+        }
+        float mean = wave_sum(s) * invC;
+        float q = 0.f;
+#pragma unroll
+        for (int i = 0; i < NV; ++i) {
+            const int c = lane * 4 + i * 256;
+            if (c < p.C) {
+                const float a = v[i].x - mean, b = v[i].y - mean, cc = v[i].z - mean, d = v[i].w - mean;
+                q += a * a + b * b + cc * cc + d * d;
+            }
+        }
+        float rstd = rsqrtf(wave_sum(q) * invC + p.eps_a);
+        if (p.stats_a != nullptr && lane == 0) p.stats_a[row] = make_float2(mean, rstd);
+        s = 0.f;
+#pragma unroll
+        for (int i = 0; i < NV; ++i) {
+            const int c = lane * 4 + i * 256;
+            if (c < p.C) {
+                const float4 g = *(const float4*)(p.gamma_a + c), b = *(const float4*)(p.beta_a + c);
+                float4 o;
+                o.x = (v[i].x - mean) * rstd * g.x + b.x;
+                o.y = (v[i].y - mean) * rstd * g.y + b.y;
+                o.z = (v[i].z - mean) * rstd * g.z + b.z;
+                o.w = (v[i].w - mean) * rstd * g.w + b.w;
+                *(float4*)(p.y + row * p.C + c) = o;
+                v[i] = o;
+                s += o.x + o.y + o.z + o.w;
+            }
+        }
+        mean = wave_sum(s) * invC;
+        q = 0.f;
+#pragma unroll
+        for (int i = 0; i < NV; ++i) {
+            const int c = lane * 4 + i * 256;
+            if (c < p.C) {
+                const float a = v[i].x - mean, b = v[i].y - mean, cc = v[i].z - mean, d = v[i].w - mean;
+                q += a * a + b * b + cc * cc + d * d;
+            }
+        }
+        rstd = rsqrtf(wave_sum(q) * invC + p.eps_b);
+        if (p.stats_b != nullptr && lane == 0) p.stats_b[row] = make_float2(mean, rstd);
+#pragma unroll
+        for (int i = 0; i < NV; ++i) {
+            const int c = lane * 4 + i * 256;
+            if (c < p.C) {
+                const float4 g = *(const float4*)(p.gamma_b + c), b = *(const float4*)(p.beta_b + c);
+                float4 o;
+                o.x = (v[i].x - mean) * rstd * g.x + b.x;
+                o.y = (v[i].y - mean) * rstd * g.y + b.y;
+                o.z = (v[i].z - mean) * rstd * g.z + b.z;
+                o.w = (v[i].w - mean) * rstd * g.w + b.w;
+                if (p.d32 != nullptr) *(float4*)(p.d32 + row * p.C + c) = o;
+                if (p.d16 != nullptr) store4(p.d16, 0, row * p.C + c, o);
+            }
+        }
+    }
+}
+
+extern "C" int uenc_layernorm2_fwd(const void* x, int x_dtype, const void* res, int res_dtype, float* h_out, const float* gamma_a,
+                                   const float* beta_a, float eps_a, float* y, float* stats_a, const float* gamma_b, const float* beta_b,
+                                   float eps_b, float* d32, void* d16, float* stats_b, long M, int C, hipStream_t stream) {
+    UENC_CHECK_ARG(x && gamma_a && beta_a && y && gamma_b && beta_b && (d32 || d16) && M > 0 && C > 0 && C % 4 == 0 && C <= 1024);
+    Ln2Fwd p;
+    p.x = x; p.x_f32 = (x_dtype == UENC_F32); p.res = res; p.res_f32 = (res_dtype == UENC_F32); p.h_out = h_out;
+    p.gamma_a = gamma_a; p.beta_a = beta_a; p.y = y; p.stats_a = (float2*)stats_a; p.eps_a = eps_a;
+    p.gamma_b = gamma_b; p.beta_b = beta_b; p.d32 = d32; p.d16 = (bf16*)d16; p.stats_b = (float2*)stats_b; p.eps_b = eps_b;
+    p.M = M; p.C = C;
+    long blocks = (M + 3) / 4;
+    if (blocks > 8192) blocks = 8192;
+    const int nv = (C + 255) / 256;
+    dim3 grid((unsigned)blocks), block(256);
+    if (nv <= 1) hipLaunchKernelGGL(ln2_fwd_kernel<1>, grid, block, 0, stream, p);
+    else if (nv <= 2) hipLaunchKernelGGL(ln2_fwd_kernel<2>, grid, block, 0, stream, p);
+    else hipLaunchKernelGGL(ln2_fwd_kernel<4>, grid, block, 0, stream, p);
+    UENC_LAUNCH_RET();
+}
+
+struct Ln2Bwd {
+    const void* dd; int dd_f32;
+    const float* y;
+    const float2* stats_b; const float* gamma_b;
+    const float* dy;
+    const void* h; int h_f32;
+    const float2* stats_a; const float* gamma_a;
+    const float* dres;
+    float* dx; bf16* dx16;
+    float* dgamma_a; float* dbeta_a; float* dgamma_b; float* dbeta_b;
+    float* part_a; float* part_b;
+    long M; int C;
+};
+
+__device__ __forceinline__ float add_rounded(float a, float b) {
+#pragma clang fp contract(off)
+    asm volatile("" : "+v"(b));
+    return a + b;
+}
+
+template <int NV>
+__device__ __forceinline__ void ln2_param_out(float* sh, const float4 (&ag)[NV], const float4 (&ab)[NV], int C, int lane, float* part,
+                                              float* dgamma, float* dbeta) {
+    float* mine = sh + (long)(threadIdx.x >> 6) * 2 * C;
+#pragma unroll
+    for (int i = 0; i < NV; ++i) {
+        const int c = lane * 4 + i * 256;
+        if (c < C) { *(float4*)(mine + c) = ag[i]; *(float4*)(mine + C + c) = ab[i]; }
+    }
+    __syncthreads();
+    for (int c = threadIdx.x; c < 2 * C; c += 256) {
+        const float v = sh[c] + sh[2 * C + c] + sh[4 * C + c] + sh[6 * C + c];
+        if (part != nullptr) part[(long)blockIdx.x * 2 * C + c] = v;
+        else atomicAdd((c < C ? dgamma + c : dbeta + (c - C)), v);
+    }
+    __syncthreads();
+}
+
+template <int NV>
+__global__ __launch_bounds__(256) void ln2_bwd_kernel(Ln2Bwd p) {
+    extern __shared__ __attribute__((aligned(16))) float sh[];
+    const int lane = threadIdx.x & 63;
+    const long wave0 = (long)blockIdx.x * 4 + (threadIdx.x >> 6);
+    const long nwaves = (long)gridDim.x * 4;
+    const float invC = 1.0f / (float)p.C;
+    float4 aga[NV], aba[NV], gma[NV], agb[NV], abb[NV], gmb[NV];
+#pragma unroll
+    for (int i = 0; i < NV; ++i) {
+        aga[i] = make_float4(0.f, 0.f, 0.f, 0.f);
+        aba[i] = aga[i]; agb[i] = aga[i]; abb[i] = aga[i];
+        const int c = lane * 4 + i * 256;
+        gma[i] = c < p.C ? *(const float4*)(p.gamma_a + c) : aga[i];
+        gmb[i] = c < p.C ? *(const float4*)(p.gamma_b + c) : aga[i];
+    }
+    for (long row = wave0; row < p.M; row += nwaves) {
+        const float2 sb = p.stats_b[row], sa = p.stats_a[row];
+        float4 d[NV], xh[NV], rs[NV], up[NV], hv[NV];
+#pragma unroll
+        for (int i = 0; i < NV; ++i) {
+            const int c = lane * 4 + i * 256;
+            if (c < p.C) {
+                if (p.dres != nullptr) rs[i] = *(const float4*)(p.dres + row * p.C + c);
+                if (p.dy != nullptr) up[i] = *(const float4*)(p.dy + row * p.C + c);
+                hv[i] = load4(p.h, p.h_f32, row * p.C + c);
+            }
+        }
+        float s1 = 0.f, s2 = 0.f;
+#pragma unroll
+        for (int i = 0; i < NV; ++i) {
+            const int c = lane * 4 + i * 256;
+            if (c < p.C) {
+                d[i] = load4(p.dd, p.dd_f32, row * p.C + c);
+                const float4 yv = *(const float4*)(p.y + row * p.C + c);
+                xh[i] = make_float4((yv.x - sb.x) * sb.y, (yv.y - sb.x) * sb.y, (yv.z - sb.x) * sb.y, (yv.w - sb.x) * sb.y);
+                agb[i].x += d[i].x * xh[i].x; agb[i].y += d[i].y * xh[i].y; agb[i].z += d[i].z * xh[i].z; agb[i].w += d[i].w * xh[i].w;
+                abb[i].x += d[i].x; abb[i].y += d[i].y; abb[i].z += d[i].z; abb[i].w += d[i].w;
+                d[i].x *= gmb[i].x; d[i].y *= gmb[i].y; d[i].z *= gmb[i].z; d[i].w *= gmb[i].w;
+                s1 += d[i].x + d[i].y + d[i].z + d[i].w;
+                s2 += d[i].x * xh[i].x + d[i].y * xh[i].y + d[i].z * xh[i].z + d[i].w * xh[i].w;
+            }
+        }
+        s1 = wave_sum(s1) * invC;
+        s2 = wave_sum(s2) * invC;
+#pragma unroll
+        for (int i = 0; i < NV; ++i) {
+            const int c = lane * 4 + i * 256;
+            if (c < p.C) {
+                float4 o;
+                o.x = sb.y * (d[i].x - s1 - xh[i].x * s2);
+                o.y = sb.y * (d[i].y - s1 - xh[i].y * s2);
+                o.z = sb.y * (d[i].z - s1 - xh[i].z * s2);
+                o.w = sb.y * (d[i].w - s1 - xh[i].w * s2);
+                if (p.dy != nullptr) {
+                    o.x = add_rounded(up[i].x, o.x); o.y = add_rounded(up[i].y, o.y);
+                    o.z = add_rounded(up[i].z, o.z); o.w = add_rounded(up[i].w, o.w);
+                }
+                d[i] = o;
+            }
+        }
+        s1 = 0.f; s2 = 0.f;
+#pragma unroll
+        for (int i = 0; i < NV; ++i) {
+            const int c = lane * 4 + i * 256;
+            if (c < p.C) {
+                xh[i] = make_float4((hv[i].x - sa.x) * sa.y, (hv[i].y - sa.x) * sa.y, (hv[i].z - sa.x) * sa.y, (hv[i].w - sa.x) * sa.y);
+                aga[i].x += d[i].x * xh[i].x; aga[i].y += d[i].y * xh[i].y; aga[i].z += d[i].z * xh[i].z; aga[i].w += d[i].w * xh[i].w;
+                aba[i].x += d[i].x; aba[i].y += d[i].y; aba[i].z += d[i].z; aba[i].w += d[i].w;
+                d[i].x *= gma[i].x; d[i].y *= gma[i].y; d[i].z *= gma[i].z; d[i].w *= gma[i].w;
+                s1 += d[i].x + d[i].y + d[i].z + d[i].w;
+                s2 += d[i].x * xh[i].x + d[i].y * xh[i].y + d[i].z * xh[i].z + d[i].w * xh[i].w;
+            }
+        }
+        s1 = wave_sum(s1) * invC;
+        s2 = wave_sum(s2) * invC;
+#pragma unroll
+        for (int i = 0; i < NV; ++i) {
+            const int c = lane * 4 + i * 256;
+            if (c < p.C) {
+                float4 o;
+                o.x = sa.y * (d[i].x - s1 - xh[i].x * s2);
+                o.y = sa.y * (d[i].y - s1 - xh[i].y * s2);
+                o.z = sa.y * (d[i].z - s1 - xh[i].z * s2);
+                o.w = sa.y * (d[i].w - s1 - xh[i].w * s2);
+                if (p.dres != nullptr) { o.x += rs[i].x; o.y += rs[i].y; o.z += rs[i].z; o.w += rs[i].w; }
+                *(float4*)(p.dx + row * p.C + c) = o;
+                if (p.dx16 != nullptr) store4(p.dx16, 0, row * p.C + c, o);
+            }
+        }
+    }
+    if (p.dgamma_a != nullptr) {
+        ln2_param_out<NV>(sh, aga, aba, p.C, lane, p.part_a, p.dgamma_a, p.dbeta_a);
+        ln2_param_out<NV>(sh, agb, abb, p.C, lane, p.part_b, p.dgamma_b, p.dbeta_b);
+    }
+}
+
+extern "C" int uenc_layernorm2_bwd(const void* dd, int dd_dtype, const float* y, const float* stats_b, const float* gamma_b, const float* dy,
+                                   const void* h, int h_dtype, const float* stats_a, const float* gamma_a, const float* dres, float* dx,
+                                   void* dx16, float* dgamma_a, float* dbeta_a, float* dgamma_b, float* dbeta_b, long M, int C,
+                                   float* part_ws_a, float* part_ws_b, int defer_param_sums, hipStream_t stream) {
+    UENC_CHECK_ARG(dd && y && stats_b && gamma_b && h && stats_a && gamma_a && dx && M > 0 && C > 0 && C % 4 == 0 && C <= 1024);
+    const bool params = dgamma_a != nullptr;
+    UENC_CHECK_ARG((dbeta_a != nullptr) == params && (dgamma_b != nullptr) == params && (dbeta_b != nullptr) == params);
+    UENC_CHECK_ARG((part_ws_a == nullptr) == (part_ws_b == nullptr) && (part_ws_a == nullptr || part_ws_a != part_ws_b));
+    Ln2Bwd p;
+    p.dd = dd; p.dd_f32 = (dd_dtype == UENC_F32); p.y = y; p.stats_b = (const float2*)stats_b; p.gamma_b = gamma_b; p.dy = dy;
+    p.h = h; p.h_f32 = (h_dtype == UENC_F32); p.stats_a = (const float2*)stats_a; p.gamma_a = gamma_a; p.dres = dres;
+    p.dx = dx; p.dx16 = (bf16*)dx16; p.dgamma_a = dgamma_a; p.dbeta_a = dbeta_a; p.dgamma_b = dgamma_b; p.dbeta_b = dbeta_b;
+    p.M = M; p.C = C;
+    bool stored = false;
+    const long blocks = ln_bwd_blocks(M, C, part_ws_a != nullptr && params, &stored);
+    p.part_a = stored ? part_ws_a : nullptr;
+    p.part_b = stored ? part_ws_b : nullptr;
+    const int nv = (C + 255) / 256;
+    const size_t shm = (size_t)4 * 2 * C * sizeof(float);
+    dim3 grid((unsigned)blocks), block(256);
+    if (nv <= 1) hipLaunchKernelGGL(ln2_bwd_kernel<1>, grid, block, shm, stream, p);
+    else if (nv <= 2) hipLaunchKernelGGL(ln2_bwd_kernel<2>, grid, block, shm, stream, p);
+    else hipLaunchKernelGGL(ln2_bwd_kernel<4>, grid, block, shm, stream, p);
+    if (stored && !defer_param_sums) {
+        const dim3 pg((2 * C + 63) / 64, 16);
+        hipLaunchKernelGGL(ln_bwd_param_kernel, pg, dim3(256), 0, stream, (const float*)p.part_a, (int)blocks, C, dgamma_a, dbeta_a);
+        hipLaunchKernelGGL(ln_bwd_param_kernel, pg, dim3(256), 0, stream, (const float*)p.part_b, (int)blocks, C, dgamma_b, dbeta_b);
+    }
+    UENC_LAUNCH_RET();
+}
diff --git a/uni-encoder-code_amd/uenc/attention.py b/uni-encoder-code_amd/uenc/attention.py
--- a/uni-encoder-code_amd/uenc/attention.py
+++ b/uni-encoder-code_amd/uenc/attention.py
@@ -25,6 +25,39 @@
     return m, m.shape[-1]
 
 
+def fwd_launch(q, k, v, m8, mrs, lse, nheads, scale, dropout_p=0.0, seed=0):
+    B, Lq, E = q.shape
+    S = k.shape[1]
+    out = torch.empty((B, Lq, E), dtype=torch.bfloat16, device=q.device)
+    nws = lib.uenc_mha_fwd_workspace_floats(B, nheads, Lq, S)
+    ws = torch.empty((nws,), dtype=torch.float32, device=q.device) if nws else None
+    args = (q.data_ptr(), q.stride(0), q.stride(1), k.data_ptr(), k.stride(0), k.stride(1),
+            v.data_ptr(), v.stride(0), v.stride(1), m8.data_ptr() if m8 is not None else 0, mrs,
+            out.data_ptr(), out.stride(0), out.stride(1), lse.data_ptr(),
+            ws.data_ptr() if ws is not None else 0, B, nheads, Lq, S, scale, float(dropout_p))
+    if isinstance(seed, K.SeedSlot):
+        check(lib.uenc_mha_fwd_sp(*args, seed.seeds.data_ptr(), seed.slot, stream_ptr()), "mha_fwd_sp")
+    else:
+        check(lib.uenc_mha_fwd(*args, int(seed), stream_ptr()), "mha_fwd")
+    return out
+
+
+def bwd_launch(q, k, v, m8, mrs, out, lse, dout, dq, dk, dv, nheads, scale, dropout_p=0.0, seed=0):
+    B, Lq, E = q.shape
+    S = k.shape[1]
+    args = (q.data_ptr(), q.stride(0), q.stride(1), k.data_ptr(), k.stride(0), k.stride(1),
+            v.data_ptr(), v.stride(0), v.stride(1), m8.data_ptr() if m8 is not None else 0, mrs,
+            out.data_ptr(), out.stride(0), out.stride(1), lse.data_ptr(),
+            dout.data_ptr(), dout.stride(0), dout.stride(1),
+            dq.data_ptr(), dq.stride(0), dq.stride(1), dk.data_ptr(), dk.stride(0), dk.stride(1),
+            dv.data_ptr(), dv.stride(0), dv.stride(1), B, nheads, Lq, S, scale, dropout_p)
+    if isinstance(seed, K.SeedSlot):
+        seed.check()
+        check(lib.uenc_mha_bwd_sp(*args, seed.seeds.data_ptr(), seed.slot, stream_ptr()), "mha_bwd_sp")
+    else:
+        check(lib.uenc_mha_bwd(*args, seed, stream_ptr()), "mha_bwd")
+
+
 class MHACoreFn(torch.autograd.Function):
     @staticmethod
     def forward(ctx, q, k, v, nheads, mask, dropout_p=0.0, seed=0):
@@ -46,17 +79,7 @@
             ctx.save_for_backward(q, k, v, out, lse, m8 if m8 is not None else torch.empty(0, device=q.device))
             ctx.meta = (nheads, S, scale, mrs, m8 is not None, float(dropout_p), int(seed))
             return out
-        out = torch.empty((B, Lq, E), dtype=torch.bfloat16, device=q.device)
-        nws = lib.uenc_mha_fwd_workspace_floats(B, nheads, Lq, S)
-        ws = torch.empty((nws,), dtype=torch.float32, device=q.device) if nws else None
-        args = (q.data_ptr(), q.stride(0), q.stride(1), k.data_ptr(), k.stride(0), k.stride(1),
-                v.data_ptr(), v.stride(0), v.stride(1), m8.data_ptr() if m8 is not None else 0, mrs,
-                out.data_ptr(), out.stride(0), out.stride(1), lse.data_ptr(),
-                ws.data_ptr() if ws is not None else 0, B, nheads, Lq, S, scale, float(dropout_p))
-        if isinstance(seed, K.SeedSlot):
-            check(lib.uenc_mha_fwd_sp(*args, seed.seeds.data_ptr(), seed.slot, stream_ptr()), "mha_fwd_sp")
-        else:
-            check(lib.uenc_mha_fwd(*args, int(seed), stream_ptr()), "mha_fwd")
+        out = fwd_launch(q, k, v, m8, mrs, lse, nheads, scale, dropout_p, seed)
         ctx.save_for_backward(q, k, v, out, lse, m8 if m8 is not None else torch.empty(0, device=q.device))
         ctx.meta = (nheads, S, scale, mrs, m8 is not None, float(dropout_p), seed if isinstance(seed, K.SeedSlot) else int(seed))
         return out
@@ -83,17 +106,7 @@
         dq = torch.zeros((B, Lq, E), dtype=torch.float32, device=q.device)
         dk = torch.empty((B, S, E), dtype=torch.bfloat16, device=q.device)
         dv = torch.empty((B, S, E), dtype=torch.bfloat16, device=q.device)
-        args = (q.data_ptr(), q.stride(0), q.stride(1), k.data_ptr(), k.stride(0), k.stride(1),
-                v.data_ptr(), v.stride(0), v.stride(1), m8.data_ptr() if has_mask else 0, mrs,
-                out.data_ptr(), out.stride(0), out.stride(1), lse.data_ptr(),
-                dout.data_ptr(), dout.stride(0), dout.stride(1),
-                dq.data_ptr(), dq.stride(0), dq.stride(1), dk.data_ptr(), dk.stride(0), dk.stride(1),
-                dv.data_ptr(), dv.stride(0), dv.stride(1), B, nheads, Lq, S, scale, dropout_p)
-        if isinstance(seed, K.SeedSlot):
-            seed.check()
-            check(lib.uenc_mha_bwd_sp(*args, seed.seeds.data_ptr(), seed.slot, stream_ptr()), "mha_bwd_sp")
-        else:
-            check(lib.uenc_mha_bwd(*args, seed, stream_ptr()), "mha_bwd")
+        bwd_launch(q, k, v, m8 if has_mask else None, mrs, out, lse, dout, dq, dk, dv, nheads, scale, dropout_p, seed)
         return dq.to(torch.bfloat16), dk, dv, None, None, None, None
 
 
diff --git a/uni-encoder-code_amd/uenc/capi.py b/uni-encoder-code_amd/uenc/capi.py
--- a/uni-encoder-code_amd/uenc/capi.py
+++ b/uni-encoder-code_amd/uenc/capi.py
@@ -48,6 +48,10 @@
     "uenc_layernorm_fwd": [c_p, c_i, c_p, c_i, c_p, c_p, c_p, c_p, c_i, c_p, c_l, c_i, c_f, c_p, c_p],
     "uenc_layernorm_bwd": [c_p, c_i, c_p, c_i, c_p, c_p, c_p, c_p, c_i, c_p, c_p, c_l, c_i, c_p, c_p, c_i, c_p],
     "uenc_layernorm_bwd_blocks": [c_l, c_i],
+    "uenc_layernorm2_fwd": [c_p, c_i, c_p, c_i, c_p, c_p, c_p, c_f, c_p, c_p, c_p, c_p, c_f, c_p, c_p, c_p, c_l, c_i, c_p],
+    "uenc_layernorm2_bwd": [c_p, c_i, c_p, c_p, c_p, c_p, c_p, c_i, c_p, c_p, c_p, c_p, c_p, c_p, c_p, c_p, c_p, c_l, c_i, c_p, c_p, c_i, c_p],
+    "uenc_gemm_nt_adda": [c_p, c_i, c_l, c_p, c_l, c_p, c_i, c_l, c_i, c_i, c_i, c_p, c_i, c_p, c_l, c_p, c_l, c_f, c_i, c_i, c_p, c_l, c_i, c_i,
+                          c_p],
     "uenc_ln_param_grouped": [c_p, c_i, c_i, c_p],
     "uenc_window_attn_bwd_groups": [c_i, c_i, c_i, c_i, c_i],
     "uenc_window_attn_dtable_grouped": [c_p, c_i, c_i, c_p],
diff --git a/uni-encoder-code_amd/uenc/kernels.py b/uni-encoder-code_amd/uenc/kernels.py
--- a/uni-encoder-code_amd/uenc/kernels.py
+++ b/uni-encoder-code_amd/uenc/kernels.py
@@ -223,6 +223,24 @@
     return out
 
 
+def gemm_nt_adda(a: torch.Tensor, a2: torch.Tensor, w: torch.Tensor, n_add: int, *, bias: Optional[torch.Tensor] = None,
+                 out_dtype=torch.bfloat16) -> torch.Tensor:
+    _mat(a, "a"); _mat(a2, "a2"); _mat(w, "w")
+    M, K = a.shape
+    N = w.shape[0]
+    if EXACT:
+        raise capi.UencError("gemm_nt_adda: bf16-operand kernels only")
+    if a.dtype != torch.float32 or a2.dtype != torch.float32 or w.dtype != torch.bfloat16 or a2.shape[1] != K or w.shape[1] != K or M % a2.shape[0]:
+        raise capi.UencError(f"gemm_nt_adda: a {tuple(a.shape)} {a.dtype} a2 {tuple(a2.shape)} {a2.dtype} w {tuple(w.shape)} {w.dtype}")
+    out = torch.empty((M, N), dtype=out_dtype, device=a.device)
+    if bias is not None:
+        assert bias.dtype == torch.float32 and bias.numel() == N and bias.is_contiguous()
+    check(lib.uenc_gemm_nt_adda(a.data_ptr(), dt(a), a.stride(0), w.data_ptr(), w.stride(0), out.data_ptr(), dt(out), out.stride(0), M, N, K,
+                                ptr(bias), EPI_NONE, None, 0, None, 0, 1.0, 1, 0, a2.data_ptr(), a2.stride(0), a2.shape[0], int(n_add),
+                                stream_ptr()), "gemm_nt_adda")
+    return out
+
+
 def _gemm_nt_exact(a, w, bias, epilogue, aux, aux_out, out, alpha, accumulate) -> torch.Tensor:
     M, K = a.shape
     N, K2 = w.shape
@@ -372,6 +390,52 @@
           "layernorm_bwd")
     if twin_exact is not None and dx_dtype == torch.float32:
         twin_exact.append(dx)
+    return dx
+
+
+def layernorm2_fwd(x: torch.Tensor, gamma_a, beta_a, gamma_b, beta_b, *, res: Optional[torch.Tensor] = None, want_h: bool = False,
+                   eps_a: float = 1e-5, eps_b: float = 1e-5, want_d32: bool = True, want_d16: bool = False):
+    C = x.shape[-1]
+    assert x.is_cuda and x.is_contiguous() and all(t.dtype == torch.float32 and t.numel() == C for t in (gamma_a, beta_a, gamma_b, beta_b))
+    assert (want_d32 or want_d16) and not (EXACT and want_d16)
+    M = x.numel() // C
+    f32 = dict(dtype=torch.float32, device=x.device)
+    if res is not None:
+        assert res.shape == x.shape and res.is_contiguous()
+    y, d32 = torch.empty(x.shape, **f32), (torch.empty(x.shape, **f32) if want_d32 else None)
+    d16 = torch.empty(x.shape, dtype=torch.bfloat16, device=x.device) if want_d16 else None
+    h = torch.empty(x.shape, **f32) if want_h else None
+    sa, sb = torch.empty((M, 2), **f32), torch.empty((M, 2), **f32)
+    check(lib.uenc_layernorm2_fwd(x.data_ptr(), dt(x), ptr(res), dt(res) if res is not None else 0, ptr(h), gamma_a.data_ptr(), beta_a.data_ptr(),
+                                  float(eps_a), y.data_ptr(), sa.data_ptr(), gamma_b.data_ptr(), beta_b.data_ptr(), float(eps_b), ptr(d32), ptr(d16),
+                                  sb.data_ptr(), M, C, stream_ptr()), "layernorm2_fwd")
+    return y, h, sa, d32, d16, sb
+
+
+def layernorm2_bwd(dd: torch.Tensor, y: torch.Tensor, stats_b, gamma_b, dy: Optional[torch.Tensor], h: torch.Tensor, stats_a, gamma_a, *,
+                   dres: Optional[torch.Tensor] = None, dgamma_a=None, dbeta_a=None, dgamma_b=None, dbeta_b=None,
+                   twin: Optional[list] = None, defer: Optional["SmallReductions"] = None) -> torch.Tensor:
+    C = h.shape[-1]
+    M = h.numel() // C
+    assert dd.is_contiguous() and y.is_contiguous() and h.is_contiguous() and dd.shape == h.shape and y.shape == h.shape and y.dtype == torch.float32
+    for t in (dy, dres):
+        if t is not None:
+            assert t.dtype == torch.float32 and t.is_contiguous() and t.shape == h.shape
+    dx = torch.empty(h.shape, dtype=torch.float32, device=h.device)
+    dx16 = None
+    if twin is not None:
+        dx16 = dx if EXACT else torch.empty(h.shape, dtype=torch.bfloat16, device=h.device)
+        twin.append(dx16)
+    pa, deferred = _ln_part(M, C, dgamma_a, dbeta_a, h.device, defer)
+    pb = None
+    if pa is not None:
+        if deferred:
+            pb, _ = _ln_part(M, C, dgamma_b, dbeta_b, h.device, defer)
+        else:
+            pb = _scratch("ln2_bwd_b", 2048 * 2 * C * 4, h.device)
+    check(lib.uenc_layernorm2_bwd(dd.data_ptr(), dt(dd), y.data_ptr(), stats_b.data_ptr(), gamma_b.data_ptr(), ptr(dy), h.data_ptr(), dt(h),
+                                  stats_a.data_ptr(), gamma_a.data_ptr(), ptr(dres), dx.data_ptr(), None if EXACT else ptr(dx16), ptr(dgamma_a),
+                                  ptr(dbeta_a), ptr(dgamma_b), ptr(dbeta_b), M, C, ptr(pa), ptr(pb), int(deferred), stream_ptr()), "layernorm2_bwd")
     return dx
 
 
diff --git a/uni-encoder-code_amd/uenc/modeling/transformer_decoder/oneformer_transformer_decoder.py b/uni-encoder-code_amd/uenc/modeling/transformer_decoder/oneformer_transformer_decoder.py
--- a/uni-encoder-code_amd/uenc/modeling/transformer_decoder/oneformer_transformer_decoder.py
+++ b/uni-encoder-code_amd/uenc/modeling/transformer_decoder/oneformer_transformer_decoder.py
@@ -63,6 +63,11 @@
         self.norm = nn.LayerNorm(d_model)
 
     def forward(self, tgt, tgt_mask=None, tgt_key_padding_mask=None, query_pos=None):
+        sa = self.self_attn
+        if (query_pos is not None and tgt_mask is None and not K.EXACT and tgt.dtype == torch.float32 and query_pos.shape == tgt.shape
+                and sa.embed_dim == 32 * sa.num_heads and not (self.training and sa.dropout > 0.0)):
+            o = ops.self_attention_core(tgt, query_pos, sa.in_proj_weight, sa.in_proj_bias, sa.num_heads)
+            return _ln(self.norm, ops.linear(o, sa.out_proj.weight, sa.out_proj.bias, residual=tgt))
         qk = tgt if query_pos is None else tgt + query_pos
         return _ln(self.norm, self.self_attn(qk, qk, tgt, attn_mask=tgt_mask, residual=tgt))
 
@@ -88,9 +93,14 @@
         self.linear2 = nn.Linear(dim_feedforward, d_model)
         self.norm = nn.LayerNorm(d_model)
 
-    def forward(self, tgt):
+    def forward(self, tgt, then_norm: Optional[nn.LayerNorm] = None):
         h = ops.mlp(tgt, [self.linear1.weight, self.linear1.bias, self.linear2.weight, self.linear2.bias], act="relu", residual=tgt)
-        return _ln(self.norm, h)
+        if then_norm is None:
+            return _ln(self.norm, h)
+        if K.EXACT or h.dtype != torch.float32 or h.shape[-1] > 1024:
+            y = _ln(self.norm, h)
+            return y, _ln(then_norm, y)
+        return ops.layer_norm2(h, self.norm.weight, self.norm.bias, then_norm.weight, then_norm.bias, eps_a=self.norm.eps, eps_b=then_norm.eps)
 
 
 class MLP(nn.Module):
@@ -305,9 +315,9 @@
             output = self.transformer_cross_attention_layers[i](output, src[lvl], memory_mask=attn_mask, query_pos=qe,
                                                                 key_in=kin[lvl])
             output = self.transformer_self_attention_layers[i](output, query_pos=qe)
-            output = self.transformer_ffn_layers[i](output)
+            output, normed = self.transformer_ffn_layers[i](output, then_norm=self.decoder_norm)
             cls, msk, attn_mask = self.forward_prediction_heads(output, (mf16, H4, W4, mes),
-                                                                size_list[(i + 1) % self.num_feature_levels])
+                                                                size_list[(i + 1) % self.num_feature_levels], normed=normed)
             predictions_class.append(cls); predictions_mask.append(msk)
         assert len(predictions_class) == self.num_layers + 1
         nq = predictions_class[0].shape[1]
@@ -318,9 +328,9 @@
                 "pred_logits": predictions_class[-1], "pred_masks": predictions_mask[-1],
                 "aux_outputs": [{"pred_logits": a, "pred_masks": b} for a, b in zip(predictions_class[:-1], predictions_mask[:-1])]}
 
-    def forward_prediction_heads(self, output, mf, attn_mask_target_size):
+    def forward_prediction_heads(self, output, mf, attn_mask_target_size, normed=None):
         mf16, H4, W4, mes = mf
-        d = _ln(self.decoder_norm, output)
+        d = normed if normed is not None else _ln(self.decoder_norm, output)
         outputs_class = d
         me = self.mask_embed(d, out_dtype=torch.bfloat16).contiguous()
         B, Q, _ = me.shape
diff --git a/uni-encoder-code_amd/uenc/ops.py b/uni-encoder-code_amd/uenc/ops.py
--- a/uni-encoder-code_amd/uenc/ops.py
+++ b/uni-encoder-code_amd/uenc/ops.py
@@ -679,6 +679,38 @@
 
 def layer_norm(x, gamma, beta, *, res=None, out_dtype=F32, eps=1e-5):
     return LayerNormFn.apply(x, res, gamma, beta, out_dtype, eps)
+
+
+class LayerNorm2Fn(torch.autograd.Function):
+
+    @staticmethod
+    def forward(ctx, x, gamma_a, beta_a, gamma_b, beta_b, eps_a, eps_b):
+        xc = x.contiguous()
+        y, _, sa, d, _, sb = K.layernorm2_fwd(xc, gamma_a.detach(), beta_a.detach(), gamma_b.detach(), beta_b.detach(), eps_a=eps_a, eps_b=eps_b)
+        ctx.save_for_backward(xc, sa, y, sb, gamma_a, beta_a, gamma_b, beta_b)
+        ctx.set_materialize_grads(False)
+        return y, d
+
+    @staticmethod
+    def backward(ctx, dy, dd):
+        h, sa, y, sb, gamma_a, beta_a, gamma_b, beta_b = ctx.saved_tensors
+        ga = (grad_buf(gamma_a), grad_buf(beta_a)) if gamma_a.requires_grad else (None, None)
+        if dd is None:
+            dx = None if dy is None else _ln_bwd(dy.contiguous(), h, sa, gamma_a.detach(), dgamma=ga[0], dbeta=ga[1])
+            _tn_notify(gamma_a, beta_a)
+            return dx, None, None, None, None, None, None
+        train = gamma_a.requires_grad and gamma_b.requires_grad
+        assert train or not (gamma_a.requires_grad or gamma_b.requires_grad), "the chained LayerNorm trains both norms or neither"
+        gb = (grad_buf(gamma_b), grad_buf(beta_b)) if train else (None, None)
+        dx = K.layernorm2_bwd(dd.contiguous(), y, sb, gamma_b.detach(), None if dy is None else dy.contiguous(), h, sa, gamma_a.detach(),
+                              dgamma_a=ga[0], dbeta_a=ga[1], dgamma_b=gb[0], dbeta_b=gb[1], defer=_defer())
+        _after_deferred()
+        _tn_notify(gamma_a, beta_a, gamma_b, beta_b)
+        return dx, None, None, None, None, None, None
+
+
+def layer_norm2(x, gamma_a, beta_a, gamma_b, beta_b, *, eps_a=1e-5, eps_b=1e-5):
+    return LayerNorm2Fn.apply(x, gamma_a, beta_a, gamma_b, beta_b, eps_a, eps_b)
 
 
 class DeviceScales:
@@ -1257,6 +1289,56 @@
     return mha(q, k, v, nheads, mask, dropout_p, seed)
 
 
+class SelfAttnCoreFn(torch.autograd.Function):
+
+    @staticmethod
+    def forward(ctx, x, pos, weight, bias, nheads):
+        from . import attention as A
+        B, L, E = x.shape
+        M = B * L
+        x2 = x.reshape(M, E)
+        x2 = x2 if x2.is_contiguous() else x2.contiguous()
+        pd = pos.detach()
+        if pd.stride(0) == 0 and pd[0].is_contiguous():
+            p2 = pd[0]
+        else:
+            p2 = pd.reshape(M, E)
+            p2 = p2 if p2.is_contiguous() else p2.contiguous()
+        qkv = K.gemm_nt_adda(x2, p2, CACHE.mat(weight), 2 * E, bias=bias.detach()).view(B, L, 3 * E)
+        lse = torch.empty((B, nheads, L), dtype=F32, device=x.device)
+        out = A.fwd_launch(qkv[..., :E], qkv[..., E:2 * E], qkv[..., 2 * E:], None, 0, lse, nheads, 32 ** -0.5)
+        ctx.save_for_backward(x2, p2, qkv, out, lse, weight, bias)
+        ctx.nheads = nheads
+        return out
+
+    @staticmethod
+    def backward(ctx, dout):
+        from . import attention as A
+        x2, p2, qkv, out, lse, weight, bias = ctx.saved_tensors
+        B, L, E3 = qkv.shape
+        E, M = E3 // 3, B * L
+        dout = A._strided(dout)
+        dq = torch.zeros((B, L, E), dtype=F32, device=qkv.device)
+        dqkv = torch.empty((B, L, E3), dtype=BF16, device=qkv.device)
+        A.bwd_launch(qkv[..., :E], qkv[..., E:2 * E], qkv[..., 2 * E:], None, 0, out, lse, dout, dq, dqkv[..., E:2 * E], dqkv[..., 2 * E:],
+                     ctx.nheads, 32 ** -0.5)
+        dqkv[..., :E].copy_(dq)
+        g = dqkv.view(M, E3)
+        dqk = _dgrad_gemm(g[:, :2 * E], weight, (0, 2 * E), out_dtype=F32)
+        dx = dqk
+        if ctx.needs_input_grad[0]:
+            dx = _dgrad_gemm(g[:, 2 * E:], weight, (2 * E, 3 * E), epilogue=K.EPI_RESIDUAL, aux=dqk, out_dtype=F32).view(B, L, E)
+        if weight.requires_grad or bias.requires_grad:
+            xp16 = K.add_cast_bf16(x2, p2)
+            _wgrad(g[:, :2 * E], xp16, weight, bias, (0, 2 * E))
+            _wgrad(g[:, 2 * E:], x2, weight, bias, (2 * E, 3 * E))
+        return (dx if ctx.needs_input_grad[0] else None), (dqk.view(B, L, E) if ctx.needs_input_grad[1] else None), None, None, None
+
+
+def self_attention_core(x, pos, weight, bias, nheads: int):
+    return SelfAttnCoreFn.apply(x, pos, weight, bias, nheads)
+
+
 class GroupNormTokensFn(torch.autograd.Function):
 
     @staticmethod
```

Result: no change. 30.56 img/s, median of 3 (+0.7%).
